# oscarkey/safe-exploration

Measured on AMD Instinct MI355X. Metric: cem_particle_step_evals_per_s, higher is better.
Workload: dtype f64

## Files before the change

safe_exploration_amd/csrc/sx_gp_rollout.hip:

```cpp
#include <hip/hip_runtime.h>

#include <algorithm>
#include <cstdlib>
#include <cstring>
#include <vector>

#include "../../include/sx_amd.h"
#include "sx_big.hpp"
#include "sx_big_launch.hpp"
#include "sx_host.hpp"
#include "sx_launch.hpp"
#include "sx_rw_launch.hpp"
#include "sx_stream_launch.hpp"

namespace sx {

#ifdef SX_STAMPS
extern unsigned long long* g_stamp_host;
#endif

struct RolloutPlan {
    int form;
    bool ok;
    size_t lds;
    int nrb;
};

struct FormOverride {
    int form;
    bool strict;
    bool refuses() const { return strict && form >= 0; }
};
static const FormOverride& form_override() {
    static const FormOverride o = [] {
        const char* e = std::getenv("SX_ROLLOUT");
        const int form = !e                            ? -1
                         : std::strcmp(e, "stream") == 0 ? SX_FORM_STREAM
                         : std::strcmp(e, "rw") == 0     ? SX_FORM_RW
                         : std::strcmp(e, "rh") == 0     ? SX_FORM_RH
                                                         : -1;
        return FormOverride{form, std::getenv("SX_ROLLOUT_STRICT") != nullptr};
    }();
    return o;
}

template <int NS, int NU>
static int resident_lds_bytes(int n_train, int n_pad, int H, size_t* rh, size_t* rw) {
    *rh = rollout_rh_lds_bytes<NS, NU>(n_train, n_pad, H);
    *rw = rollout_rw_lds_bytes<NS, NU>(n_train, n_pad, H);
    return SX_OK;
}
static int resident_lds_bytes(int ns, int nu, int n_train, int n_pad, int H, size_t* rh, size_t* rw) {
#define CALL(NS, NU) resident_lds_bytes<NS, NU>(n_train, n_pad, H, rh, rw)
    SX_DISPATCH(ns, nu, CALL);
#undef CALL
}

static RolloutPlan plan_rollout(const sx_gp_model* m, int sh, int H, bool elites, bool stream_only = false) {
    const int ns = m->n_s, nu = m->n_u - sh, n_train = m->n_train, n_pad = m->n_pad;
    auto stream_lds = [&](bool byout) { return rollout_stream_lds_bytes(ns, nu, sh, n_train, n_pad, H, byout); };
    const bool all_at_once = n_pad <= 1024 && stream_lds(false) <= kMaxLdsBytes;
    const bool by_output = !all_at_once && ns > 1 && n_pad <= 1024 && stream_lds(true) <= kMaxLdsBytes;
    bool ok = rollout_compiled(ns, nu, sh);
    if (!all_at_once && !by_output) return {SX_FORM_BIG, ok && sh == 0 && !elites, 0, 0};
    if (elites && 2 * H * nu > 256 + 256 * ns) ok = false;
    if (by_output) return {SX_FORM_BYOUT, ok, stream_lds(true), 0};
    const RolloutPlan stream{SX_FORM_STREAM, ok, stream_lds(false), 0};
    const FormOverride& o = form_override();
    if (!ok || sh > 0 || stream_only || o.form == SX_FORM_STREAM) return stream;
    size_t rh, rw;
    resident_lds_bytes(ns, nu, n_train, n_pad, H, &rh, &rw);
    if (o.form != SX_FORM_RW && rh <= kMaxLdsBytes) return {SX_FORM_RH, true, rh, n_pad >> 4};
    if (o.form != SX_FORM_RH && rw <= kMaxLdsBytes) return {SX_FORM_RW, true, rw, n_pad >> 4};
    return {SX_FORM_STREAM, !o.refuses(), stream.lds, 0};
}

template <int NS, int NU, int SH>
static int launch_rollout(const sx_gp_model* m, const sx_env* env, const RolloutPtrs& rp, double* workspace,
                          int64_t workspace_bytes, hipStream_t stream) {
    RolloutPlan plan = plan_rollout(m, SH, rp.H, rp.elite_rows != nullptr);
    if (!plan.ok) return SX_ERR_UNSUPPORTED;
    if constexpr (SH == 0) {
        if (plan.form == SX_FORM_BIG) return launch_rollout_big<NS, NU>(m, env, rp, workspace, workspace_bytes, stream);
    }
    ReachConst<NS, NU> rc;
    CostConst<SX_MAX_M, NS, NU> cc;
    if (int r = env_consts<NS, NU>(env, rc, cc)) return r;
    RolloutPtrs rps = rp;
#ifdef SX_STAMPS
    rps.stamps = g_stamp_host;
#endif
    if constexpr (SH == 0) {
        if (plan.form == SX_FORM_RH || plan.form == SX_FORM_RW) {
            const int r = plan.form == SX_FORM_RH
                              ? launch_rollout_rh<NS, NU>(make_gp_const<NS, NU>(m, 8), rc, cc, rps, plan.nrb, plan.lds, stream)
                              : launch_rollout_rw<NS, NU>(make_gp_const<NS, NU>(m, kRwWaves), rc, cc, rps, plan.nrb, plan.lds,
                                                          stream);
            if (r != SX_ERR_UNSUPPORTED || form_override().refuses()) return r;
            plan = {SX_FORM_STREAM, true, rollout_stream_lds_bytes(NS, NU, SH, m->n_train, m->n_pad, rp.H, false), 0};
        }
    }
    return launch_rollout_stream<NS, NU, SH>(make_gp_const<NS, NU + SH>(m, kRolloutThreads / 64), rc, cc, rps,
                                             plan.form == SX_FORM_BYOUT, plan.lds, stream);
}

static RolloutPlan plan_rollout_multi(const sx_gp_model* models, int E, int H, bool elites) {
    RolloutPlan out{SX_FORM_STREAM, true, 0, 0};
    for (int i = 0; i < E; ++i) {
        const RolloutPlan p = plan_rollout(&models[i], 0, H, elites, true);
        if (p.form == SX_FORM_BIG || !p.ok) return {p.form, false, 0, 0};
        if (p.form == SX_FORM_BYOUT) out.form = SX_FORM_BYOUT;
    }
    const sx_gp_model& m0 = models[0];
    for (int i = 0; i < E; ++i)
        out.lds = std::max(out.lds, rollout_stream_lds_bytes(m0.n_s, m0.n_u, 0, models[i].n_train, models[i].n_pad, H,
                                                             out.form == SX_FORM_BYOUT));
    return out;
}

template <int NS, int NU>
static int64_t gp_table_entry_bytes() {
    return (int64_t)sizeof(GpConst<NS, NS + NU>);
}
static int64_t gp_table_entry_bytes(int ns, int nu) {
#define CALL(NS, NU) gp_table_entry_bytes<NS, NU>()
    SX_DISPATCH(ns, nu, CALL);
#undef CALL
}

template <int NS, int NU>
static int build_gp_table(const sx_gp_model* models, int E, void* table, hipStream_t stream) {
    std::vector<GpConst<NS, NS + NU>> host(E);
    for (int i = 0; i < E; ++i) host[i] = make_gp_const<NS, NU>(&models[i], kRolloutThreads / 64);
    return copy_model_table(host, table, stream);
}

template <int NS, int NU>
static int launch_rollout_multi(const sx_gp_model* models, const void* table, const sx_env* env, const RolloutPtrs& rp,
                                hipStream_t stream) {
    const RolloutPlan plan = plan_rollout_multi(models, rp.E, rp.H, rp.elite_rows != nullptr);
    if (!plan.ok) return SX_ERR_UNSUPPORTED;
    ReachConst<NS, NU> rc;
    CostConst<SX_MAX_M, NS, NU> cc;
    if (int r = env_consts<NS, NU>(env, rc, cc)) return r;
    return launch_rollout_stream_multi<NS, NU>(static_cast<const GpConst<NS, NS + NU>*>(table), rc, cc, rp,
                                               plan.form == SX_FORM_BYOUT, plan.lds, stream);
}

static int cem_rollout(const sx_gp_model* model, const sx_env* env, int query_shift, const RolloutPtrs& rp, void* workspace,
                       int64_t workspace_bytes, void* stream) {
#define CALL(NS, NU, SH) launch_rollout<NS, NU, SH>(model, env, rp, (double*)workspace, workspace_bytes, (hipStream_t)stream)
    SX_ROLLOUT_DISPATCH(env->n_s, env->n_u, query_shift, CALL);
#undef CALL
}

}

extern "C" {

int64_t sx_cem_rollout_workspace_bytes(const sx_gp_model* model, int E, int P, int H) {
    if (!model || E <= 0 || P <= 0 || H <= 0) return -1;
    if (sx::plan_rollout(model, 0, H, false).form != SX_FORM_BIG) return 0;
    return sx::big_ws_layout(nullptr, model->n_s, model->n_s + model->n_u, model->n_pad, (int64_t)E * P).total *
           (int64_t)sizeof(double);
}

int sx_cem_rollout_form(const sx_gp_model* model, int H) {
    if (!model || H <= 0) return -1;
    const sx::RolloutPlan plan = sx::plan_rollout(model, 0, H, false);
    return plan.ok ? plan.form : -1;
}

int sx_cem_rollout(const sx_gp_model* model, const sx_env* env, int E, int P, int H, const double* x0, const double* q0,
                   const double* mean, const double* std, const double* noise, double* actions, double* traj,
                   double* sigma, double* obj_cost, double* con_cost, int32_t* status, void* workspace,
                   int64_t workspace_bytes, void* stream) {
    return sx_cem_rollout_junk(model, env, 0, E, P, H, x0, q0, mean, std, noise, actions, traj, sigma, obj_cost, con_cost,
                               status, workspace, workspace_bytes, stream);
}

int sx_cem_rollout_elites(const sx_gp_model* model, const sx_env* env, int E, int P, int H, const double* x0, const double* q0,
                          const double* elite_rows, int k, const double* noise, double* actions, double* traj, double* sigma,
                          double* obj_cost, double* con_cost, int32_t* status, double* mean_out, double* std_out, void* stream) {
    return sx_cem_rollout_elites_junk(model, env, 0, E, P, H, x0, q0, elite_rows, k, noise, actions, traj, sigma, obj_cost,
                                      con_cost, status, mean_out, std_out, stream);
}

static sx::RolloutPtrs with_elites(sx::RolloutPtrs rp, const double* elite_rows, int k, double* mean_out, double* std_out) {
    rp.elite_rows = elite_rows;
    rp.elite_k = k;
    rp.mean_out = mean_out;
    rp.std_out = std_out;
    return rp;
}

static bool rollout_shapes_ok(const sx_gp_model* model, const sx_env* env, int query_shift) {
    return model->n_s == env->n_s && query_shift >= 0 && query_shift <= env->n_u && model->n_u == env->n_u + query_shift;
}

int sx_cem_rollout_junk(const sx_gp_model* model, const sx_env* env, int query_shift, int E, int P, int H, const double* x0,
                        const double* q0, const double* mean, const double* std, const double* noise, double* actions,
                        double* traj, double* sigma, double* obj_cost, double* con_cost, int32_t* status, void* workspace,
                        int64_t workspace_bytes, void* stream) {
    const sx::RolloutPtrs rp{x0, q0, mean, std, noise, actions, traj, sigma, obj_cost, con_cost, status, E, P, H};
    if (!model || !sx::rollout_args_ok(env, rp) || !rollout_shapes_ok(model, env, query_shift)) return SX_ERR_ARG;
    return sx::cem_rollout(model, env, query_shift, rp, workspace, workspace_bytes, stream);
}

int sx_cem_rollout_elites_junk(const sx_gp_model* model, const sx_env* env, int query_shift, int E, int P, int H,
                               const double* x0, const double* q0, const double* elite_rows, int k, const double* noise,
                               double* actions, double* traj, double* sigma, double* obj_cost, double* con_cost,
                               int32_t* status, double* mean_out, double* std_out, void* stream) {
    const sx::RolloutPtrs rp = with_elites({x0, q0, nullptr, nullptr, noise, actions, traj, sigma, obj_cost, con_cost, status,
                                            E, P, H}, elite_rows, k, mean_out, std_out);
    if (!model || !elite_rows || !sx::rollout_args_ok(env, rp) || !rollout_shapes_ok(model, env, query_shift)) return SX_ERR_ARG;
    return sx::cem_rollout(model, env, query_shift, rp, nullptr, 0, stream);
}

static bool multi_models_ok(const sx_gp_model* models, int E) {
    if (!models || E <= 0) return false;
    const int ns = models[0].n_s, nu = models[0].n_u;
    if (ns <= 0 || ns > SX_MAX_NS || nu <= 0 || nu > SX_MAX_NU) return false;
    for (int i = 0; i < E; ++i)
        if (models[i].n_s != ns || models[i].n_u != nu || models[i].n_train <= 0 || models[i].n_pad <= 0) return false;
    return true;
}

int64_t sx_gp_model_table_bytes(int n_s, int n_u, int E) {
    if (E <= 0 || n_s <= 0 || n_s > SX_MAX_NS || n_u <= 0 || n_u > SX_MAX_NU) return -1;
    const int64_t entry = sx::gp_table_entry_bytes(n_s, n_u);
    return entry == SX_ERR_UNSUPPORTED ? -1 : entry * E;
}

int sx_gp_model_table(const sx_gp_model* models, int E, void* table, void* stream) {
    if (!table || !multi_models_ok(models, E)) return SX_ERR_ARG;
    for (int i = 0; i < E; ++i)
        if (!models[i].x_train || !models[i].a_pack || !models[i].stage_tab) return SX_ERR_ARG;
#define CALL(NS, NU) sx::build_gp_table<NS, NU>(models, E, table, (hipStream_t)stream)
    SX_DISPATCH(models[0].n_s, models[0].n_u, CALL);
#undef CALL
}

int sx_cem_rollout_multi_form(const sx_gp_model* models, int E, int H) {
    if (!multi_models_ok(models, E) || H <= 0) return -1;
    const sx::RolloutPlan plan = sx::plan_rollout_multi(models, E, H, false);
    return plan.ok ? plan.form : -1;
}

static int cem_rollout_multi(const sx_gp_model* models, const void* table, const sx_env* env, const sx::RolloutPtrs& rp,
                             void* stream) {
#define CALL(NS, NU) sx::launch_rollout_multi<NS, NU>(models, table, env, rp, (hipStream_t)stream)
    SX_DISPATCH(env->n_s, env->n_u, CALL);
#undef CALL
}

int sx_cem_rollout_multi(const sx_gp_model* models, const void* table, const sx_env* env, int E, int P, int H,
                         const double* x0, const double* q0, const double* mean, const double* std, const double* noise,
                         double* actions, double* traj, double* sigma, double* obj_cost, double* con_cost, int32_t* status,
                         void* stream) {
    const sx::RolloutPtrs rp{x0, q0, mean, std, noise, actions, traj, sigma, obj_cost, con_cost, status, E, P, H};
    if (!table || !sx::rollout_args_ok(env, rp) || !multi_models_ok(models, E)) return SX_ERR_ARG;
    if (models[0].n_s != env->n_s || models[0].n_u != env->n_u) return SX_ERR_ARG;
    return cem_rollout_multi(models, table, env, rp, stream);
}

int sx_cem_rollout_elites_multi(const sx_gp_model* models, const void* table, const sx_env* env, int E, int P, int H,
                                const double* x0, const double* q0, const double* elite_rows, int k, const double* noise,
                                double* actions, double* traj, double* sigma, double* obj_cost, double* con_cost,
                                int32_t* status, double* mean_out, double* std_out, void* stream) {
    const sx::RolloutPtrs rp = with_elites({x0, q0, nullptr, nullptr, noise, actions, traj, sigma, obj_cost, con_cost, status,
                                            E, P, H}, elite_rows, k, mean_out, std_out);
    if (!table || !elite_rows || !sx::rollout_args_ok(env, rp) || !multi_models_ok(models, E)) return SX_ERR_ARG;
    if (models[0].n_s != env->n_s || models[0].n_u != env->n_u) return SX_ERR_ARG;
    return cem_rollout_multi(models, table, env, rp, stream);
}

}
```

safe_exploration_amd/csrc/sx_rollout_rh.hpp:

```cpp
#pragma once
#include <hip/hip_runtime.h>

#include "../../include/sx_amd.h"
#include "sx_rollout_rw.hpp"

#ifndef SX_RH_REGP
#define SX_RH_REGP 26
#endif
#ifndef SX_RH_LEAD
#define SX_RH_LEAD -1
#endif
#ifndef SX_RH_LDSP
#define SX_RH_LDSP 8
#endif
#ifndef SX_RH_PFG
#define SX_RH_PFG 6
#endif
#ifndef SX_RH_PFL
#define SX_RH_PFL 2
#endif
#ifndef SX_RH_RBMAJOR
#define SX_RH_RBMAJOR 1
#endif
#ifndef SX_RH_PRIO
#define SX_RH_PRIO 0
#endif
#ifndef SX_RH_WFIRST
#define SX_RH_WFIRST 0
#endif
#ifndef SX_RH_SHARES
#define SX_RH_SHARES 4, 4, 4, 1, 4, 4, 4
#endif

namespace sx {

constexpr int kRhWaves = 8;
constexpr int kRhThreads = 64 * kRhWaves;

template <int NS, int NRB>
struct RhPlan {
    int wave_of[NS][NRB];
    int pairs[kRhWaves];
    constexpr RhPlan() : wave_of{}, pairs{} {
        for (int w = 0; w < kRhWaves; ++w) pairs[w] = 0;
        for (int d = 0; d < NS; ++d) {
            int lo = 0, n = kRhWaves;
            if (kRhWaves % NS == 0) {
                n = kRhWaves / NS;
                lo = d * n;
            }
            const bool rev = (kRhWaves % NS == 0) && (d & 1);
            int set_of[NRB] = {};
            int load[kRhWaves] = {};
            for (int rb = NRB - 1; rb >= 0; --rb) {
                int best = 0;
                for (int s = 1; s < n; ++s)
                    if (load[s] + pairs[lo + (rev ? n - 1 - s : s)] < load[best] + pairs[lo + (rev ? n - 1 - best : best)]) best = s;
                set_of[rb] = best;
                load[best] += 2 * (rb + 1);
            }
            for (int rb = 0; rb < NRB; ++rb) wave_of[d][rb] = lo + (rev ? n - 1 - set_of[rb] : set_of[rb]);
            for (int s = 0; s < n; ++s) pairs[lo + (rev ? n - 1 - s : s)] += load[s];
        }
    }
    constexpr int max_pairs() const {
        int m = 0;
        for (int w = 0; w < kRhWaves; ++w) m = pairs[w] > m ? pairs[w] : m;
        return m;
    }
    constexpr bool has(int w, int d) const {
        for (int rb = 0; rb < NRB; ++rb)
            if (wave_of[d][rb] == w) return true;
        return false;
    }
    constexpr int qmax(int w, int d) const {
        for (int rb = NRB - 1; rb >= 0; --rb)
            if (wave_of[d][rb] == w) return 2 * (rb + 1);
        return 0;
    }
};

template <int NS, int NRB>
struct RhElements {
    static constexpr int kMax = NS * NRB * (NRB + 1);
    short d[kRhWaves][kMax], rb[kRhWaves][kMax], q[kRhWaves][kMax];
    int n[kRhWaves];
    constexpr RhElements() : d{}, rb{}, q{}, n{} {
        const RhPlan<NS, NRB> plan{};
        for (int w = 0; w < kRhWaves; ++w) {
            int idx = 0;
            for (int dd = 0; dd < NS; ++dd) {
#if SX_RH_RBMAJOR
                for (int r = NRB - 1; r >= 0; --r)
                    for (int qq = 0; qq < 2 * (r + 1); ++qq)
                        if (plan.wave_of[dd][r] == w) { d[w][idx] = dd; rb[w][idx] = r; q[w][idx] = qq; ++idx; }
#else
                for (int qq = 0; qq < 2 * NRB; ++qq)
                    for (int r = NRB - 1; r >= 0; --r)
                        if (plan.wave_of[dd][r] == w && qq < 2 * (r + 1)) { d[w][idx] = dd; rb[w][idx] = r; q[w][idx] = qq; ++idx; }
#endif
            }
            n[w] = idx;
        }
    }
};

struct RhLayout {
    int nr, nl, ng, lead;
    constexpr RhLayout(int total, int regp, int ldsp)
        : nr(total < regp ? total : regp), nl(0), ng(0), lead(0) {
        nl = total - nr < ldsp ? total - nr : ldsp;
        ng = total - nr - nl;
        lead = SX_RH_LEAD < 0 || ng == 0 ? nr : (SX_RH_LEAD < nr ? SX_RH_LEAD : nr);
    }
    constexpr int storage(int e, int regp, int ldsp) const {
        if (SX_RH_LEAD < 0 || ng == 0) return e;
        if (e < lead) return e;
        if (e < lead + ng) return regp + ldsp + (e - lead);
        if (e < lead + ng + nl) return regp + (e - lead - ng);
        return lead + (e - lead - ng - nl);
    }
};

template <int NS, int NRB, int MAXP, int REGP, int LDSP>
struct RhStream {
    int pair[kRhWaves][MAXP];
    constexpr RhStream() : pair{} {
        const RhElements<NS, NRB> el{};
        constexpr int wpo = NRB * (NRB + 1);
        for (int w = 0; w < kRhWaves; ++w) {
            const RhLayout lay(el.n[w], REGP, LDSP);
            for (int i = 0; i < MAXP; ++i) pair[w][i] = 0;
            for (int e = 0; e < el.n[w]; ++e)
                pair[w][lay.storage(e, REGP, LDSP)] = el.d[w][e] * wpo + el.rb[w][e] * (el.rb[w][e] + 1) + el.q[w][e];
        }
    }
};

enum RhOpKind { kRhLoadB = 0, kRhLoadWL = 1, kRhLoadWG = 2, kRhMfma = 3, kRhRowEpi = 4, kRhFinalEpi = 5 };
struct RhOp {
    int kind;
    int i;
    int rb;
    int q;
    int d;
    int slot;
    int e;
};
template <int NS, int NRB, int WAVE, int REGP, int LDSP, int PF, int PFL, int PFG>
struct RhProgram {
    static constexpr int kMaxOps = 4 * NS * NRB * (NRB + 1) / 2 + 8 * NRB * NS + 16;
    RhOp ops[kMaxOps];
    int n;
    int total;
    constexpr RhProgram() : ops{}, n(0), total(0) {
        const RhElements<NS, NRB> el{};
        total = el.n[WAVE];
        const RhLayout lay(total, REGP, LDSP);
        int next_l = 0;
        int next_g = 0;
        const int e_g0 = (SX_RH_LEAD < 0 || lay.ng == 0) ? lay.nr + lay.nl : lay.lead;
        const int e_l0 = (SX_RH_LEAD < 0 || lay.ng == 0) ? lay.nr : lay.lead + lay.ng;
        int bslot[RhElements<NS, NRB>::kMax] = {};
        int bfirst[RhElements<NS, NRB>::kMax] = {};
        int nloads = 0;
        for (int e = 0; e < total; ++e) {
            const bool fresh = SX_RH_RBMAJOR || e == 0 || el.q[WAVE][e] != el.q[WAVE][e - 1] || el.d[WAVE][e] != el.d[WAVE][e - 1];
            if (fresh) ++nloads;
            bfirst[e] = fresh ? 1 : 0;
            bslot[e] = (nloads - 1) % (PF + 1);
        }
        constexpr int kDelay = 2;
        int pend_rb[NRB * NS] = {}, pend_d[NRB * NS] = {}, pend_at[NRB * NS] = {};
        int npend = 0, done = 0;
        int issued_b = 0;
        int eb = 0;
        auto issue_b_upto = [&](int loads_wanted) {
            while (issued_b < loads_wanted && eb < total) {
                if (bfirst[eb]) {
                    ops[n++] = RhOp{kRhLoadB, 0, 0, el.q[WAVE][eb], el.d[WAVE][eb], bslot[eb]};
                    ++issued_b;
                }
                ++eb;
            }
        };
        int loads_seen = 0;
        for (int e = 0; e < total; ++e) {
            if (bfirst[e]) ++loads_seen;
            issue_b_upto(loads_seen + PF);
            while (next_l < lay.nl && e_l0 + next_l <= e + PFL) ops[n++] = RhOp{kRhLoadWL, REGP + next_l++, 0, 0, 0, 0};
            while (next_g < lay.ng && e_g0 + next_g <= e + PFG) ops[n++] = RhOp{kRhLoadWG, REGP + LDSP + next_g++, 0, 0, 0, 0};
            ops[n++] = RhOp{kRhMfma, lay.storage(e, REGP, LDSP), el.rb[WAVE][e], el.q[WAVE][e], el.d[WAVE][e], bslot[e], e};
            const bool last_of_rb = el.q[WAVE][e] == 2 * (el.rb[WAVE][e] + 1) - 1;
            if (last_of_rb) {
                pend_rb[npend] = el.rb[WAVE][e];
                pend_d[npend] = el.d[WAVE][e];
                pend_at[npend] = e + kDelay;
                ++npend;
            }
            while (done < npend && pend_at[done] <= e) {
                ops[n++] = RhOp{kRhRowEpi, 0, pend_rb[done], 0, pend_d[done], 0};
                ++done;
            }
        }
        while (done < npend) {
            ops[n++] = RhOp{kRhRowEpi, 0, pend_rb[done], 0, pend_d[done], 0};
            ++done;
        }
        const RhPlan<NS, NRB> plan{};
        for (int d = 0; d < NS; ++d)
            if (plan.has(WAVE, d)) ops[n++] = RhOp{kRhFinalEpi, 0, 0, 0, d, 0};
    }
};

template <int NS, int D, int NRB, int WAVE, int REGP, int LDSP>
__device__ __forceinline__ void rh_mfma_phase(const GpConst<NS, D>& gc, GpTileLds<NS, D>& lds, const v2d* wlds_wave, int lane,
                                              const v2d (&wreg)[REGP]) {
    constexpr int PF = SX_RW_PF, PFL = SX_RH_PFL, PFG = SX_RH_PFG;
    constexpr int MAXP = RhPlan<NS, NRB>{}.max_pairs();
    static constexpr RhProgram<NS, NRB, WAVE, REGP, LDSP, PF, PFL, PFG> prog{};
    static constexpr RhStream<NS, NRB, MAXP, REGP, LDSP> stream{};
    const v2d* kbase = reinterpret_cast<const v2d*>(lds.kfrag) + lane;
    typedef const __attribute__((address_space(1))) v2d* gv2d;
    typedef const __attribute__((address_space(3))) v2d* lv2d;
    const v2d* ap_opaque = reinterpret_cast<const v2d*>(gc.a_pack) + lane;
    asm volatile("" : "+v"(ap_opaque));
    const gv2d ap = (gv2d)ap_opaque;
    const lv2d wl_base = (lv2d)wlds_wave + lane;
    v4d acc[NRB];
    v2d b[PF + 1];
    v2d wl[PFL + 1];
    v2d wg[PFG + 1];
    double ssq[NS];
#pragma unroll
    for (int d = 0; d < NS; ++d) ssq[d] = 0.0;
    static_for<0, prog.n>([&](auto ktag) {
        constexpr RhOp op = prog.ops[decltype(ktag)::value];
        if constexpr (op.kind == kRhLoadB) {
            b[op.slot] = kbase[(op.q * NS + op.d) * 64];
        } else if constexpr (op.kind == kRhLoadWL) {
            wl[op.i % (PFL + 1)] = wl_base[(op.i - REGP) * 64];
        } else if constexpr (op.kind == kRhLoadWG) {
            wg[op.i % (PFG + 1)] = ap[(size_t)stream.pair[WAVE][op.i] * 64];
        } else if constexpr (op.kind == kRhMfma) {
#if SX_RH_PRIO == 2
            if constexpr ((4 * op.e) / prog.total != (4 * (op.e - 1)) / prog.total || op.e == 0)
                __builtin_amdgcn_s_setprio(3 - (4 * op.e) / prog.total);
#endif
            SX_PIN();
            const v2d bq = b[op.slot];
            v2d a;
            if constexpr (op.i < REGP)
                a = wreg[op.i];
            else if constexpr (op.i < REGP + LDSP)
                a = wl[op.i % (PFL + 1)];
            else
                a = wg[op.i % (PFG + 1)];
            if constexpr (op.q == 0)
                acc[op.rb] = __builtin_amdgcn_mfma_f64_16x16x4f64(a.x, bq.x, v4d{0.0, 0.0, 0.0, 0.0}, 0, 0, 0);
            else
                acc[op.rb] = __builtin_amdgcn_mfma_f64_16x16x4f64(a.x, bq.x, acc[op.rb], 0, 0, 0);
            acc[op.rb] = __builtin_amdgcn_mfma_f64_16x16x4f64(a.y, bq.y, acc[op.rb], 0, 0, 0);
            SX_PIN();
        } else if constexpr (op.kind == kRhRowEpi) {
            constexpr int rb = op.rb, d = op.d;
            double s;
            if constexpr (rb >= NRB - 2) {
                const int row0 = rb * 16 + (lane >> 4);
                s = 0.0;
#pragma unroll
                for (int r = 0; r < 4; ++r) {
                    const int row = row0 + 4 * r;
                    if (row < gc.n_train)
                        s = fma(acc[rb][r], acc[rb][r], s);
                    else if (row - gc.n_train <= D)
                        lds.mj[d * 256 + (row - gc.n_train) * 16 + (lane & 15)] = acc[rb][r];
                }
            } else {
                s = fma(acc[rb][3], acc[rb][3], fma(acc[rb][2], acc[rb][2], fma(acc[rb][1], acc[rb][1], acc[rb][0] * acc[rb][0])));
            }
            ssq[d] += s;
        } else {
            constexpr int d = op.d;
            const v4d tot = __builtin_amdgcn_mfma_f64_16x16x4f64(1.0, ssq[d], v4d{0.0, 0.0, 0.0, 0.0}, 0, 0, 0);
            if (lane < 16) lds.part[(WAVE * NS + d) * 16 + lane] = tot[0];
        }
    });
}

template <int NS, int D, int NRB, bool WITH_JAC, typename G>
__device__ __forceinline__ void rh_collect(const G& gc, const GpTileLds<NS, D>& lds, int c, const double (&z)[D],
                                           double (&mean)[NS], double (&var)[NS], double (&jac)[NS][D]) {
    constexpr RhPlan<NS, NRB> plan{};
#pragma unroll
    for (int d = 0; d < NS; ++d) {
        double q = 0.0;
#pragma unroll
        for (int w = 0; w < kRhWaves; ++w)
            if (plan.has(w, d)) q += lds.part[(w * NS + d) * 16 + c];
        var[d] = (gc.outputscale[d] - q) + gc.noise[d];
        const double m = lds.mj[d * 256 + c];
        mean[d] = m;
        if constexpr (WITH_JAC) {
#pragma unroll
            for (int j = 0; j < D; ++j) jac[d][j] = lds.mj[d * 256 + (1 + j) * 16 + c] - z[j] * gc.inv_ls2[d * D + j] * m;
        }
    }
}

template <int NS, int NRB>
constexpr int rh_regp() {
    constexpr int m = RhPlan<NS, NRB>{}.max_pairs();
    return m < SX_RH_REGP ? m : SX_RH_REGP;
}
template <int NS, int NRB>
constexpr int rh_ldsp() {
    constexpr int rest = RhPlan<NS, NRB>{}.max_pairs() - rh_regp<NS, NRB>();
    return rest < SX_RH_LDSP ? rest : SX_RH_LDSP;
}
template <int NS, int NU, int NRB>
inline size_t rh_lds_doubles(int n_train, int n_pad, int H) {
    constexpr int D = NS + NU, S = NS + NS * NS;
    return (size_t)NS * n_pad * 16 + NS * 256 + (size_t)kRhWaves * NS * 16 + 32 * D + (((size_t)SX_TILE * H * NU + 1) & ~(size_t)1) +
           (((size_t)SX_TILE * (2 * (S + NS) + 3) + 1) & ~(size_t)1) + RwKstarLds<NS, D>::doubles(n_pad) +
           (size_t)kRhWaves * rh_ldsp<NS, NRB>() * 128;
}

template <int NS, int NU, int NRB>
__global__ __launch_bounds__(kRhThreads) void cem_rollout_rh_kernel(GpConst<NS, NS + NU> gc, ReachConst<NS, NU> rc,
                                                                    CostConst<SX_MAX_M, NS, NU> cc, RolloutPtrs rp) {
    constexpr int D = NS + NU;
    constexpr int S = NS + NS * NS;
    constexpr int PQS = S + NS;
    constexpr RhPlan<NS, NRB> plan{};
    constexpr int MAXP = plan.max_pairs();
    constexpr int REGP = rh_regp<NS, NRB>();
    constexpr int LDSP = rh_ldsp<NS, NRB>();
    extern __shared__ __attribute__((aligned(16))) double smem[];
    GpTileLds<NS, D> lds;
    constexpr int nw = kRhWaves;
    lds.xs = nullptr;
    lds.etab = nullptr;
    lds.kfrag = smem;
    lds.mj = lds.kfrag + (size_t)NS * gc.n_pad * 16;
    lds.part = lds.mj + NS * 256;
    lds.zs = lds.part + (size_t)nw * NS * 16;
    double* acts = lds.zs + 32 * D;
    const int tid = threadIdx.x;
    const int wave = __builtin_amdgcn_readfirstlane(tid >> 6), lane = tid & 63;
    const int H = rp.H;
    const int tiles_per_problem = (rp.P + SX_TILE - 1) / SX_TILE;
    const int total_tiles = rp.E * tiles_per_problem;

    RwConst<NS, NU>* const cst = reinterpret_cast<RwConst<NS, NU>*>(acts + (((size_t)SX_TILE * rp.H * NU + 1) & ~(size_t)1));
    double* const pq = reinterpret_cast<double*>(cst + 1);
    RwKstarLds<NS, D> kl;
    kl.carve(pq + (((size_t)SX_TILE * (2 * PQS + 3) + 1) & ~(size_t)1), gc.n_pad);
    v2d* const wlds = reinterpret_cast<v2d*>(kl.xbar + ((D + 1) & ~1));

    static constexpr RhStream<NS, NRB, MAXP, REGP, LDSP> stream{};
    v2d wreg[REGP];
#if SX_RH_WFIRST
    {
        const v2d* __restrict__ const ap0 = reinterpret_cast<const v2d*>(gc.a_pack) + lane;
#pragma unroll
        for (int i = 0; i < REGP; ++i) wreg[i] = ap0[(size_t)stream.pair[wave][i] * 64];
        if constexpr (LDSP > 0) {
#pragma unroll
            for (int i = 0; i < LDSP; ++i) wlds[(wave * LDSP + i) * 64 + lane] = ap0[(size_t)stream.pair[wave][REGP + i] * 64];
        }
    }
#endif
    {
        static_assert(sizeof(RwConst<NS, NU>) % 8 == 0 && sizeof(ReachConst<NS, NU>) % 8 == 0 &&
                      sizeof(CostConst<SX_MAX_M, NS, NU>) % 8 == 0, "copied in 8-byte words");
        constexpr int nrc = sizeof(ReachConst<NS, NU>) / 8, ncc = sizeof(CostConst<SX_MAX_M, NS, NU>) / 8;
        double* dst = reinterpret_cast<double*>(cst);
        const double* src_rc = reinterpret_cast<const double*>(&rc);
        const double* src_cc = reinterpret_cast<const double*>(&cc);
        for (int i = tid; i < nrc; i += kRhThreads) dst[i] = src_rc[i];
        for (int i = tid; i < ncc; i += kRhThreads) dst[nrc + i] = src_cc[i];
        if (tid < NS * D) cst->inv_ls2[tid] = gc.inv_ls2[tid];
        if (tid < NS) {
            cst->outputscale[tid] = gc.outputscale[tid];
            cst->noise[tid] = gc.noise[tid];
        }
    }
    const RwConst<NS, NU>& fc = *cst;
    const ReachConst<NS, NU>& frc = cst->rc;
    const CostConst<SX_MAX_M, NS, NU>& fcc = cst->cc;
    rw_kstar_setup(gc, kl, lds.kfrag);
    const int kstar_pairs = (gc.n_train + 7) >> 3;

    const bool owner = tid < SX_TILE;
    int q0_begin, q0_end, q_begin = 0, q_end = 0;
    kstar_pair_range(kstar_pairs, wave, 1, nw, q0_begin, q0_end);
    if (wave > 0) {
        constexpr int kShare[8] = {0, SX_RH_SHARES};
        int before = 0, total = 0;
#pragma unroll
        for (int w = 1; w < 8; ++w) {
            if (w < wave) before += kShare[w];
            total += kShare[w];
        }
        kstar_pair_range(kstar_pairs, before, kShare[wave], total, q_begin, q_end);
    }
    double* const zs_base = lds.zs;

    for (int tile = blockIdx.x; tile < total_tiles; tile += gridDim.x) {
#ifdef SX_STAMPS
        const unsigned long long tile_t0 = stamp();
        unsigned long long first_k = 0, first_kb = 0;
#endif
        const int e = tile / tiles_per_problem;
        const int c0 = (tile - e * tiles_per_problem) * SX_TILE;
        const bool valid = owner && (c0 + tid < rp.P);

        const double* dist_mean = rp.mean + (int64_t)e * H * NU;
        const double* dist_std = rp.std + (int64_t)e * H * NU;
        bool have_q = rp.q0 != nullptr;
        if (rp.elite_rows) {
            const int L = H * NU, W = 2 + L;
            double* const ms = lds.kfrag;
            const double* rows = rp.elite_rows + (int64_t)e * rp.elite_k * W + 2;
            const bool publish = c0 == 0 && rp.mean_out;
            int cshift = 0;
            while ((nw << cshift) < L && cshift < 6) ++cshift;
            const int ccol = lane & ((1 << cshift) - 1);
            for (int cb = wave << cshift; cb < L; cb += nw << cshift) {
                const int col = cb + ccol;
                double m, sd;
                wave_refit_columns(rows + (col < L ? col : L - 1), rp.elite_k, W, lane, cshift, m, sd);
                if ((lane >> cshift) == 0 && col < L) {
                    ms[col] = m;
                    ms[L + col] = sd;
                    if (publish) {
                        rp.mean_out[(int64_t)e * L + col] = m;
                        rp.std_out[(int64_t)e * L + col] = sd;
                    }
                }
            }
            __syncthreads();
            dist_mean = ms;
            dist_std = ms + L;
        }
        for (int i = tid; i < SX_TILE * H * NU; i += kRhThreads) {
            const int c = i / (H * NU);
            const int r = i - c * (H * NU);
            double a = 0.0;
            if (c0 + c < rp.P) {
                const int64_t gi = ((int64_t)e * rp.P + c0 + c) * (H * NU) + r;
                if (rp.noise) {
                    a = dist_mean[r] + dist_std[r] * rp.noise[gi];
                    rp.actions[gi] = a;
                } else {
                    a = rp.actions[gi];
                }
            }
            acts[i] = a;
        }
        const bool lane_owner = lane < SX_TILE;
        const bool lane_valid = lane_owner && (c0 + lane < rp.P);
        auto st_row = [&](int buf, int c) { return pq + (buf * SX_TILE + c) * PQS; };
        double* const ac_row = pq + 2 * SX_TILE * PQS + (lane_owner ? lane : 0) * 3;
        if (owner) {
            double* my = st_row(0, tid);
#pragma unroll
            for (int i = 0; i < NS; ++i) {
                my[i] = rp.x0[(int64_t)e * NS + i];
#pragma unroll
                for (int j = 0; j < NS; ++j) my[NS + i * NS + j] = have_q ? rp.q0[((int64_t)e * NS + i) * NS + j] : 0.0;
            }
            ac_row[0] = 0.0;
            ac_row[1] = 0.0;
            reinterpret_cast<int*>(ac_row + 2)[0] = 0;
        }
        __syncthreads();
        if (owner) {
            const double* my = st_row(0, tid);
#pragma unroll
            for (int i = 0; i < NS; ++i) lds.zs[tid * D + i] = my[i];
#pragma unroll
            for (int cidx = 0; cidx < NU; ++cidx) lds.zs[tid * D + NS + cidx] = acts[(tid * H + 0) * NU + cidx];
        }
        __syncthreads();

        if (!SX_RH_WFIRST && tile == (int)blockIdx.x) {
            const v2d* __restrict__ const ap = reinterpret_cast<const v2d*>(gc.a_pack) + lane;
            if constexpr (LDSP > 0) {
                const __amdgpu_buffer_rsrc_t arsrc =
                    __builtin_amdgcn_make_buffer_rsrc(const_cast<double*>(gc.a_pack), 0, (int)0xffffffffu, 0x00020000);
#pragma unroll
                for (int i = 0; i < LDSP; ++i) {
                    const int pair = __builtin_amdgcn_readfirstlane(stream.pair[wave][REGP + i]);
                    __builtin_amdgcn_raw_ptr_buffer_load_lds(
                        arsrc, (__attribute__((address_space(3))) void*)(wlds + (wave * LDSP + i) * 64), 16, lane * 16, pair << 10, 0, 0);
                }
            }
#pragma unroll
            for (int i = 0; i < REGP; ++i) wreg[i] = ap[(size_t)stream.pair[wave][i] * 64];
        }

        auto next_centre = [&](const ReachConst<NS, NU>& R, int c, const double* z_prev, double (&out)[NS]) {
#pragma unroll
            for (int i = 0; i < NS; ++i) {
                double s = lds.mj[i * 256 + c];
#pragma unroll
                for (int j = 0; j < NS; ++j) s = fma(R.a[i * NS + j], z_prev[j], s);
#pragma unroll
                for (int cidx = 0; cidx < NU; ++cidx) s = fma(R.b[i * NU + cidx], z_prev[NS + cidx], s);
                out[i] = s;
            }
        };
        auto finish_state = [&](int t) {
            double z[D], u[NU], mean[NS], var[NS], jac[NS][D], p1[NS], Q1[NS][NS];
            double p[NS], Q[NS][NS];
            constexpr RhPlan<NS, NRB> plan{};
            const double* my = st_row(t & 1, lane);
            double partv[NS][kRhWaves], mjv[NS][1 + D], ils2[NS][D], osc[NS], nzv[NS];
#pragma unroll
            for (int d = 0; d < NS; ++d) {
#pragma unroll
                for (int w = 0; w < kRhWaves; ++w) partv[d][w] = plan.has(w, d) ? lds.part[(w * NS + d) * 16 + lane] : 0.0;
#pragma unroll
                for (int r = 0; r < 1 + D; ++r) mjv[d][r] = lds.mj[d * 256 + r * 16 + lane];
            }
#pragma unroll
            for (int i = 0; i < NS; ++i) {
                p[i] = my[i];
#pragma unroll
                for (int j = 0; j < NS; ++j) Q[i][j] = my[NS + i * NS + j];
            }
#pragma unroll
            for (int cidx = 0; cidx < NU; ++cidx) u[cidx] = acts[(lane * H + t) * NU + cidx];
#pragma unroll
            for (int d = 0; d < NS; ++d) {
                osc[d] = fc.outputscale[d];
                nzv[d] = fc.noise[d];
#pragma unroll
                for (int j = 0; j < D; ++j) ils2[d][j] = fc.inv_ls2[d * D + j];
            }
            SX_PIN();
            const ReachConst<NS, NU>& rcv = frc;
#pragma unroll
            for (int j = 0; j < NS; ++j) z[j] = p[j];
#pragma unroll
            for (int cidx = 0; cidx < NU; ++cidx) z[NS + cidx] = u[cidx];
#pragma unroll
            for (int d = 0; d < NS; ++d) {
                double q = 0.0;
#pragma unroll
                for (int w = 0; w < kRhWaves; ++w)
                    if (plan.has(w, d)) q += partv[d][w];
                var[d] = (osc[d] - q) + nzv[d];
                mean[d] = mjv[d][0];
#pragma unroll
                for (int j = 0; j < D; ++j) jac[d][j] = mjv[d][1 + j] - z[j] * ils2[d][j] * mean[d];
            }
            int st_step = 0;
            if (have_q) {
                reach_ellipsoid<NS, NU>(rcv, p, Q, u, mean, var, jac, p1, Q1, st_step);
            } else {
                reach_point<NS, NU>(rcv, p, u, mean, var, p1, Q1, st_step);
            }
            have_q = true;
            {
                double zt[D];
#pragma unroll
                for (int j = 0; j < NS; ++j) zt[j] = p[j];
#pragma unroll
                for (int cidx = 0; cidx < NU; ++cidx) zt[NS + cidx] = u[cidx];
#pragma unroll
                for (int i = 0; i < NS; ++i) {
                    double sc = mean[i];
#pragma unroll
                    for (int j = 0; j < NS; ++j) sc = fma(rcv.a[i * NS + j], zt[j], sc);
#pragma unroll
                    for (int cidx = 0; cidx < NU; ++cidx) sc = fma(rcv.b[i * NU + cidx], zt[NS + cidx], sc);
                    p1[i] = sc;
                }
                if (t + 1 < H) {
                    double* zn = zs_base + ((t + 1) & 1) * 16 * D + lane * D;
#pragma unroll
                    for (int i = 0; i < NS; ++i) zn[i] = p1[i];
#pragma unroll
                    for (int cidx = 0; cidx < NU; ++cidx) zn[NS + cidx] = acts[(lane * H + t + 1) * NU + cidx];
                }
            }
            if (lane_valid && st_step) reinterpret_cast<int*>(ac_row + 2)[0] |= st_step;
            double* nx = st_row((t + 1) & 1, lane);
#pragma unroll
            for (int i = 0; i < NS; ++i) {
                nx[i] = p1[i];
#pragma unroll
                for (int j = 0; j < NS; ++j) nx[NS + i * NS + j] = Q1[i][j];
                nx[S + i] = var[i];
            }
        };
        auto finish_costs = [&](int t) {
            const int c = lane & 15;
            const double* o = st_row((t + 1) & 1, c);
            double pp[NS], QQ[NS][NS], var[NS], hrow[NS], hv, uu[NU], umin[NU], umax[NU], wab[NS], tgt[NS], wli[NS];
            const int m = fcc.m, obj_mode = fcc.obj_mode, con_mode = fcc.con_mode;
            const int r0 = lane >> 4;
            const int r0c = r0 < m ? r0 : 0;
#pragma unroll
            for (int i = 0; i < NS; ++i) {
                pp[i] = o[i];
#pragma unroll
                for (int j = 0; j < NS; ++j) QQ[i][j] = o[NS + i * NS + j];
                var[i] = o[S + i];
                hrow[i] = fcc.h_mat[r0c * NS + i];
                wab[i] = fcc.w_abs[i];
                tgt[i] = fcc.target[i];
                wli[i] = fcc.w_lin[i];
            }
            hv = fcc.h_vec[r0c];
#pragma unroll
            for (int cidx = 0; cidx < NU; ++cidx) {
                uu[cidx] = acts[(c * H + t) * NU + cidx];
                umin[cidx] = fcc.u_min[cidx];
                umax[cidx] = fcc.u_max[cidx];
            }
            double obj = ac_row[0], con = ac_row[1];
            SX_PIN();
            bool viol = false;
            if (con_mode == SX_CON_ALL_STATES || t == H - 1) {
                for (int r = r0; r < m; r += 4) {
                    if (r != r0) {
#pragma unroll
                        for (int i = 0; i < NS; ++i) hrow[i] = fcc.h_mat[r * NS + i];
                        hv = fcc.h_vec[r];
                    }
                    double hc = 0.0, hq = 0.0;
#pragma unroll
                    for (int i = 0; i < NS; ++i) {
                        hc += hrow[i] * pp[i];
                        double sacc = 0.0;
#pragma unroll
                        for (int j = 0; j < NS; ++j) sacc += QQ[i][j] * hrow[j];
                        hq += hrow[i] * sacc;
                    }
                    const double dist = hc + sqrt(hq) - hv;
                    viol = viol || (dist >= 0.0);
                }
            }
            unsigned long long bits = __ballot(viol);
            bits |= bits >> 32;
            bits |= bits >> 16;
            if (lane_owner) {
                if ((bits >> lane) & 1ull) con += SX_STATE_VIOLATION_COST;
                bool uviol = false;
#pragma unroll
                for (int cidx = 0; cidx < NU; ++cidx) uviol = uviol || (uu[cidx] < umin[cidx]) || (uu[cidx] > umax[cidx]);
                if (uviol) con += SX_ACTION_VIOLATION_COST;
                double oadd = 0.0;
                if (obj_mode == SX_OBJ_NEG_VARIANCE) {
#pragma unroll
                    for (int i = 0; i < NS; ++i) oadd -= var[i];
                } else {
#pragma unroll
                    for (int i = 0; i < NS; ++i) oadd += wab[i] * fabs(tgt[i] - pp[i]) + wli[i] * pp[i];
                }
                obj += oadd;
                ac_row[0] = obj;
                ac_row[1] = con;
                const int64_t g = (int64_t)e * rp.P + c0 + lane;
                if (lane_valid && rp.traj) {
                    double* tr = rp.traj + (g * H + t) * S;
#pragma unroll
                    for (int i = 0; i < NS; ++i) {
                        tr[i] = pp[i];
#pragma unroll
                        for (int j = 0; j < NS; ++j) tr[NS + i * NS + j] = QQ[i][j];
                    }
                }
                if (lane_valid && rp.sigma) {
#pragma unroll
                    for (int i = 0; i < NS; ++i) rp.sigma[(g * H + t) * NS + i] = var[i];
                }
            }
        };

#ifdef SX_STAMPS
        unsigned long long c_k = 0, c_kb = 0, c_m = 0, c_mb = 0;
        unsigned long long rt0;
        asm volatile("s_memrealtime %0\n\ts_waitcnt lgkmcnt(0)" : "=s"(rt0)::"memory");
        const unsigned long long ct0 = stamp();
#endif
        for (int t = 0; t < H; ++t) {
#ifdef SX_STAMPS
            const unsigned long long t0 = stamp();
#endif
            const bool kstar_wave = !(t > 0 && wave == 0);
            if (wave == 4 && t > 1) finish_costs(t - 2);
            if (kstar_wave) {
                double zq[D];
                const int c = lane & 15;
                if (t == 0) {
#pragma unroll
                    for (int j = 0; j < D; ++j) zq[j] = zs_base[c * D + j];
                    rw_kstar_phase(gc, kl, lds.kfrag, q0_begin, q0_end, zq);
                } else {
                    double pc[NS];
                    next_centre(rc, c, zs_base + ((t - 1) & 1) * 16 * D + c * D, pc);
#pragma unroll
                    for (int i = 0; i < NS; ++i) zq[i] = pc[i];
#pragma unroll
                    for (int cidx = 0; cidx < NU; ++cidx) zq[NS + cidx] = acts[(c * H + t) * NU + cidx];
                    rw_kstar_phase(gc, kl, lds.kfrag, q_begin, q_end, zq);
                }
            } else if (owner) {
                finish_state(t - 1);
            }
#ifdef SX_STAMPS
            const unsigned long long t1 = stamp();
#endif
            if (t == 0) asm volatile("s_waitcnt vmcnt(0)" ::: "memory");
            __syncthreads();
#ifdef SX_STAMPS
            const unsigned long long t2 = stamp();
#endif
            const v2d* wl = wlds + wave * LDSP * 64;
#if SX_RH_PRIO == 1
            if (wave < 4) __builtin_amdgcn_s_setprio(3);
#endif
            switch (wave) {
                case 0: rh_mfma_phase<NS, D, NRB, 0, REGP, LDSP>(gc, lds, wl, lane, wreg); break;
                case 1: rh_mfma_phase<NS, D, NRB, 1, REGP, LDSP>(gc, lds, wl, lane, wreg); break;
                case 2: rh_mfma_phase<NS, D, NRB, 2, REGP, LDSP>(gc, lds, wl, lane, wreg); break;
                case 3: rh_mfma_phase<NS, D, NRB, 3, REGP, LDSP>(gc, lds, wl, lane, wreg); break;
                case 4: rh_mfma_phase<NS, D, NRB, 4, REGP, LDSP>(gc, lds, wl, lane, wreg); break;
                case 5: rh_mfma_phase<NS, D, NRB, 5, REGP, LDSP>(gc, lds, wl, lane, wreg); break;
                case 6: rh_mfma_phase<NS, D, NRB, 6, REGP, LDSP>(gc, lds, wl, lane, wreg); break;
                default: rh_mfma_phase<NS, D, NRB, 7, REGP, LDSP>(gc, lds, wl, lane, wreg); break;
            }
#if SX_RH_PRIO == 1
            if (wave < 4) __builtin_amdgcn_s_setprio(0);
#elif SX_RH_PRIO == 2
            __builtin_amdgcn_s_setprio(0);
#endif
#ifdef SX_STAMPS
            const unsigned long long t3 = stamp();
#endif
            __syncthreads();
#ifdef SX_STAMPS
            const unsigned long long t4 = stamp();
            c_k += t1 - t0; c_kb += t2 - t1; c_m += t3 - t2; c_mb += t4 - t3;
            if (t == 0) { first_k = t1 - t0; first_kb = t2 - t1; }
#endif
        }
#ifdef SX_STAMPS
        const unsigned long long loop_t1 = stamp();
        if (rp.stamps && lane == 0 && tile == (int)blockIdx.x) {
            unsigned long long* o = rp.stamps + ((size_t)blockIdx.x * nw + wave) * 8;
            o[0] = c_k; o[1] = c_kb; o[2] = c_m; o[3] = c_mb;
            o[4] = (ct0 - tile_t0) | (first_k << 32);
            unsigned long long rt1;
            asm volatile("s_memrealtime %0\n\ts_waitcnt lgkmcnt(0)" : "=s"(rt1)::"memory");
            o[6] = stamp() - ct0;
            o[7] = rt1 - rt0;
        }
#endif
        if (wave == 0 && owner) finish_state(H - 1);
        if (wave == 4 && H > 1) finish_costs(H - 2);
        __syncthreads();
        if (wave == 0) finish_costs(H - 1);
        if (valid) {
            const int64_t g = (int64_t)e * rp.P + c0 + tid;
            rp.obj_cost[g] = ac_row[0];
            rp.con_cost[g] = ac_row[1];
            const int st = reinterpret_cast<const int*>(ac_row + 2)[0];
            if (st) atomicOr(rp.status, st);
        }
        __syncthreads();
#ifdef SX_STAMPS
        if (rp.stamps && lane == 0 && tile == (int)blockIdx.x)
            rp.stamps[((size_t)blockIdx.x * nw + wave) * 8 + 5] = (stamp() - loop_t1) | (first_kb << 32);
#endif
    }
}

}
```

safe_exploration_amd/csrc/sx_rollout_rw.hpp:

```cpp
#pragma once
#include <hip/hip_runtime.h>

#include "../../include/sx_amd.h"
#include "sx_exp2_tab2048.hpp"
#include "sx_gp.hpp"
#include "sx_reach.hpp"
#include "sx_refit.hpp"
#include "sx_rollout.hpp"
#include "sx_rw_launch.hpp"

#ifndef SX_RW_LDSCONST
#define SX_RW_LDSCONST 1
#endif
#ifndef SX_RW_POLYLANES
#define SX_RW_POLYLANES 1
#endif
#ifndef SX_RW_PF
#define SX_RW_PF 2
#endif
#ifndef SX_RW_RCLOCAL
#define SX_RW_RCLOCAL 0
#endif
#ifndef SX_RW_POLYFOLD
#define SX_RW_POLYFOLD 0
#endif

namespace sx {

constexpr int kRwThreads = 64 * kRwWaves;
constexpr int kRwMaxPairs = 93;

template <int B, int E, typename F>
__device__ __forceinline__ void static_for(F&& f) {
    if constexpr (B < E) {
        f(std::integral_constant<int, B>{});
        static_for<B + 1, E>(f);
    }
}

template <int NS, int NRB>
struct RwPlan {
    int wave_of[NS][NRB];
    int pairs[kRwWaves];
    constexpr RwPlan() : wave_of{}, pairs{} {
        for (int w = 0; w < kRwWaves; ++w) pairs[w] = 0;
        for (int rb = NRB - 1; rb >= 0; --rb)
            for (int d = 0; d < NS; ++d) {
                int lo = 0, hi = kRwWaves;
                if (kRwWaves % NS == 0) {
                    lo = d * (kRwWaves / NS);
                    hi = lo + kRwWaves / NS;
                }
                int best = lo;
                for (int w = lo + 1; w < hi; ++w)
                    if (pairs[w] < pairs[best]) best = w;
                wave_of[d][rb] = best;
                pairs[best] += 2 * (rb + 1);
            }
    }
    constexpr int max_pairs() const {
        int m = 0;
        for (int w = 0; w < kRwWaves; ++w) m = pairs[w] > m ? pairs[w] : m;
        return m;
    }
    constexpr bool has(int w, int d) const {
        for (int rb = 0; rb < NRB; ++rb)
            if (wave_of[d][rb] == w) return true;
        return false;
    }
    constexpr int qmax(int w, int d) const {
        for (int rb = NRB - 1; rb >= 0; --rb)
            if (wave_of[d][rb] == w) return 2 * (rb + 1);
        return 0;
    }
};

template <int NS, int NRB>
constexpr bool rw_fits() {
    return RwPlan<NS, NRB>{}.max_pairs() <= kRwMaxPairs;
}

template <int NS, int NRB, int MAXP>
struct RwLoadTab {
    int pair[kRwWaves][MAXP];
    constexpr RwLoadTab() : pair{} {
        const RwPlan<NS, NRB> plan{};
        constexpr int wpo = NRB * (NRB + 1);
        for (int w = 0; w < kRwWaves; ++w) {
            int idx = 0;
            for (int d = 0; d < NS; ++d)
                for (int rb = NRB - 1; rb >= 0; --rb) {
                    if (plan.wave_of[d][rb] != w) continue;
                    for (int q = 0; q < 2 * (rb + 1); ++q) pair[w][idx++] = d * wpo + rb * (rb + 1) + q;
                }
            for (; idx < MAXP; ++idx) pair[w][idx] = 0;
        }
    }
};

template <int NS, int D, int NRB, int MAXP>
__device__ __forceinline__ void rw_load_w(const GpConst<NS, D>& gc, int wave, int lane, v2d (&wreg)[MAXP]) {
    static constexpr RwLoadTab<NS, NRB, MAXP> tab{};
    const v2d* __restrict__ ap = reinterpret_cast<const v2d*>(gc.a_pack) + lane;
#pragma unroll
    for (int i = 0; i < MAXP; ++i) wreg[i] = ap[(size_t)tab.pair[wave][i] * 64];
}

template <int NS, int D, int NRB, int WAVE, int MAXP, int PF = SX_RW_PF>
__device__ __forceinline__ void rw_mfma_phase(const GpConst<NS, D>& gc, GpTileLds<NS, D>& lds, int lane,
                                              const v2d (&wreg)[MAXP]) {
    constexpr RwPlan<NS, NRB> plan{};
    const v2d* kbase = reinterpret_cast<const v2d*>(lds.kfrag) + lane;
    int first[NS][NRB];
    {
        int idx = 0;
#pragma unroll
        for (int d = 0; d < NS; ++d)
#pragma unroll
            for (int rb = NRB - 1; rb >= 0; --rb) {
                first[d][rb] = idx;
                if (plan.wave_of[d][rb] == WAVE) idx += 2 * (rb + 1);
            }
    }
    static_for<0, NS>([&](auto dtag) {
        constexpr int d = decltype(dtag)::value;
        constexpr int qmax = plan.qmax(WAVE, d);
        if constexpr (qmax > 0) {
        v4d acc[NRB];
        v2d b[PF + 1];
#pragma unroll
        for (int q = 0; q < PF && q < qmax; ++q) b[q] = kbase[(q * NS + d) * 64];
#pragma unroll
        for (int q = 0; q < qmax; ++q) {
            if (q + PF < qmax) b[(q + PF) % (PF + 1)] = kbase[((q + PF) * NS + d) * 64];
            SX_PIN();
            const v2d bq = b[q % (PF + 1)];
#pragma unroll
            for (int rb = NRB - 1; rb >= 0; --rb) {
                if (plan.wave_of[d][rb] != WAVE || q >= 2 * (rb + 1)) continue;
                const v2d a = wreg[first[d][rb] + q];
                if (q == 0)
                    acc[rb] = __builtin_amdgcn_mfma_f64_16x16x4f64(a.x, bq.x, v4d{0.0, 0.0, 0.0, 0.0}, 0, 0, 0);
                else
                    acc[rb] = __builtin_amdgcn_mfma_f64_16x16x4f64(a.x, bq.x, acc[rb], 0, 0, 0);
                acc[rb] = __builtin_amdgcn_mfma_f64_16x16x4f64(a.y, bq.y, acc[rb], 0, 0, 0);
            }
            SX_PIN();
        }
        double ssq = 0.0;
#pragma unroll
        for (int rb = NRB - 1; rb >= 0; --rb) {
            if (plan.wave_of[d][rb] != WAVE) continue;
            double s;
            if (rb >= NRB - 2) {
                const int row0 = rb * 16 + (lane >> 4);
                s = 0.0;
#pragma unroll
                for (int r = 0; r < 4; ++r) {
                    const int row = row0 + 4 * r;
                    if (row < gc.n_train)
                        s = fma(acc[rb][r], acc[rb][r], s);
                    else if (row - gc.n_train <= D)
                        lds.mj[d * 256 + (row - gc.n_train) * 16 + (lane & 15)] = acc[rb][r];
                }
            } else {
                s = fma(acc[rb][3], acc[rb][3], fma(acc[rb][2], acc[rb][2], fma(acc[rb][1], acc[rb][1], acc[rb][0] * acc[rb][0])));
            }
            ssq += s;
        }
        const v4d tot = __builtin_amdgcn_mfma_f64_16x16x4f64(1.0, ssq, v4d{0.0, 0.0, 0.0, 0.0}, 0, 0, 0);
        if (lane < 16) lds.part[(WAVE * NS + d) * 16 + lane] = tot[0];
        }
    });
}

constexpr double kExpScale2 = 2048.0 / 0.693147180559945309417232;
constexpr double kExpUnit2 = 0.693147180559945309417232 / 2048.0;

template <int NS, int D>
struct RwKstarLds {
    double* rows;
    double* tab;
    double* xbar;
    static __host__ __device__ size_t doubles(int n_pad) { return (size_t)n_pad * (D + NS) + (n_pad & 1) + kExpTab2 + 2 + ((D + 1) & ~1); }
    __device__ void carve(double* base, int n_pad) {
        rows = base;
        tab = rows + (size_t)n_pad * (D + NS) + (n_pad & 1);
        xbar = tab + kExpTab2 + 2;
    }
};

template <int NS, int D>
__device__ __forceinline__ void rw_kstar_setup(const GpConst<NS, D>& gc, const RwKstarLds<NS, D>& kl, double* kfrag) {
    const int tid = threadIdx.x, lane = tid & 63;
    double xb[D];
#pragma unroll
    for (int j = 0; j < D; ++j) {
        double v = lane < gc.n_train ? gc.x_train[lane * D + j] : 0.0;
        for (int off = 32; off > 0; off >>= 1) v += __shfl_xor(v, off);
        xb[j] = v / (double)(gc.n_train < 64 ? gc.n_train : 64);
        if (tid == 0) kl.xbar[j] = xb[j];
    }
    for (int k = tid; k < gc.n_pad; k += blockDim.x) {
        double xr[D], cc[NS];
#pragma unroll
        for (int d = 0; d < NS; ++d) cc[d] = 0.0;
#pragma unroll
        for (int j = 0; j < D; ++j) {
            xr[j] = k < gc.n_train ? gc.x_train[k * D + j] - xb[j] : 0.0;
#pragma unroll
            for (int d = 0; d < NS; ++d) cc[d] = fma(gc.k_nh_ils2[d * D + j], xr[j] * xr[j], cc[d]);
        }
#pragma unroll
        for (int j = 0; j < D; ++j) kl.rows[k * (D + NS) + j] = xr[j];
#pragma unroll
        for (int d = 0; d < NS; ++d) kl.rows[k * (D + NS) + D + d] = cc[d];
    }
    for (int i = tid; i < kExpTab2; i += blockDim.x) kl.tab[i] = kExp2Tab2048[i];
    if (tid < 2) kl.tab[kExpTab2 + tid] = __builtin_nan("");
    const int first_pad = ((gc.n_train + 7) >> 3) * NS * 128;
    for (int i = first_pad + tid; i < (gc.n_pad >> 3) * NS * 128; i += blockDim.x) kfrag[i] = 0.0;
}

template <int NS, int D>
__device__ __forceinline__ void rw_kstar_phase(const GpConst<NS, D>& gc, const RwKstarLds<NS, D>& kl, double* kfrag,
                                               int q_begin, int q_end, const double (&z)[D]) {
    constexpr int M = 2 * NS, RS = D + NS;
    const int n = q_end - q_begin;
    if (n <= 0) return;
    const int lane = (int)threadIdx.x & 63;
    const int c = lane & 15;
    double zz[NS], g[NS][D];
    bool znan = false;
    {
        double zc[D];
#pragma unroll
        for (int j = 0; j < D; ++j) {
            zc[j] = z[j] - kl.xbar[j];
            znan = znan || (z[j] != z[j]);
        }
#pragma unroll
        for (int d = 0; d < NS; ++d) {
            double a = gc.k_log_os[d];
#pragma unroll
            for (int j = 0; j < D; ++j) {
                const double kz = gc.k_nh_ils2[d * D + j] * zc[j];
                a = fma(kz, zc[j], a);
                g[d][j] = -2.0 * kz;
            }
            zz[d] = a;
        }
    }
    const lds_f64* etab = (const lds_f64*)kl.tab + (znan ? kExpTab2 : 0);
    const int emask = znan ? 0 : kExpTab2 - 1;
    const int k0 = 8 * q_begin + (lane >> 4);
    const lds_f64* x = (const lds_f64*)kl.rows + k0 * RS;
    lds_f64* f = (lds_f64*)kfrag + kfrag_index(NS, c, k0, 0);

    struct Set {
        double t[M], p[M];
        int mi[M];
    };
    auto load_x = [&](double (&xx)[2 * RS]) {
        asm volatile("" : "+v"(x));
#pragma unroll
        for (int h = 0; h < 2; ++h)
#pragma unroll
            for (int j = 0; j < RS; ++j) xx[h * RS + j] = x[h * 4 * RS + j];
        x += 8 * RS;
    };
    auto stage_a1 = [&](const double (&xx)[2 * RS], Set& s) {
        double yc[M], m[M];
#pragma unroll
        for (int h = 0; h < 2; ++h)
#pragma unroll
            for (int d = 0; d < NS; ++d) {
                double a = xx[h * RS + D + d] + zz[d];
#pragma unroll
                for (int j = 0; j < D; ++j) a = fma(g[d][j], xx[h * RS + j], a);
                yc[h * NS + d] = a;
            }
#pragma unroll
        for (int i = 0; i < M; ++i) yc[i] = __builtin_fmax(yc[i], -800.0 * kExpScale2);
#pragma unroll
        for (int i = 0; i < M; ++i) m[i] = __builtin_rint(yc[i]);
#pragma unroll
        for (int i = 0; i < M; ++i) asm("v_cvt_i32_f64 %0, %1" : "=v"(s.mi[i]) : "v"(m[i]));
#pragma unroll
        for (int i = 0; i < M; ++i) s.t[i] = etab[s.mi[i] & emask];
#pragma unroll
#if SX_RW_POLYFOLD
        for (int i = 0; i < M; ++i) s.p[i] = yc[i] - m[i];
#else
        for (int i = 0; i < M; ++i) s.p[i] = (yc[i] - m[i]) * kExpUnit2;
#endif
    };
    auto stage_a2 = [&](Set& s) {
        double r[M];
#pragma unroll
        for (int i = 0; i < M; ++i) r[i] = s.p[i];
#pragma unroll
#if SX_RW_POLYFOLD
        for (int i = 0; i < M; ++i) s.p[i] = fma(r[i], kExpUnit2 * kExpUnit2 * kExpUnit2 / 6.0, kExpUnit2 * kExpUnit2 * 0.5);
#pragma unroll
        for (int i = 0; i < M; ++i) s.p[i] = fma(s.p[i], r[i], kExpUnit2);
#else
        for (int i = 0; i < M; ++i) s.p[i] = fma(r[i], 1.66666666666666666667e-01, 0.5);
#pragma unroll
        for (int i = 0; i < M; ++i) s.p[i] = fma(s.p[i], r[i], 1.0);
#endif
#pragma unroll
        for (int i = 0; i < M; ++i) s.p[i] = s.p[i] * r[i];
    };
    auto stage_b = [&](const Set& s) {
        asm volatile("" : "+v"(f));
        double val[M];
#pragma unroll
        for (int i = 0; i < M; ++i) val[i] = ldexp(fma(s.t[i], s.p[i], s.t[i]), s.mi[i] >> 11);
#pragma unroll
        for (int d = 0; d < NS; ++d) {
            f[d * 128] = val[d];
            f[d * 128 + 1] = val[NS + d];
        }
        f += NS * 128;
    };
    double xr[2 * RS];
    Set s0, s1;
    load_x(xr);
    stage_a1(xr, s0);
    load_x(xr);
    stage_a2(s0);
    auto body = [&](const Set& sold, Set& snew) {
        stage_a1(xr, snew);
        SX_PIN();
        load_x(xr);
        stage_b(sold);
        SX_PIN();
        stage_a2(snew);
        SX_PIN();
    };
    const int n1 = n - 1;
    for (int k = 0; k < (n1 >> 1); ++k) {
        body(s0, s1);
        body(s1, s0);
    }
    if (n1 & 1) {
        body(s0, s1);
        stage_b(s1);
    } else {
        stage_b(s0);
    }
}

template <int NS, int NU>
struct alignas(16) RwConst {
    ReachConst<NS, NU> rc;
    CostConst<SX_MAX_M, NS, NU> cc;
    double inv_ls2[NS * (NS + NU)];
    double outputscale[NS];
    double noise[NS];
};

template <int NS, int D, int NRB, bool WITH_JAC, typename G>
__device__ __forceinline__ void rw_collect(const G& gc, const GpTileLds<NS, D>& lds, int c,
                                           const double (&z)[D], double (&mean)[NS], double (&var)[NS],
                                           double (&jac)[NS][D]) {
    constexpr RwPlan<NS, NRB> plan{};
#pragma unroll
    for (int d = 0; d < NS; ++d) {
        double q = 0.0;
#pragma unroll
        for (int w = 0; w < kRwWaves; ++w)
            if (plan.has(w, d)) q += lds.part[(w * NS + d) * 16 + c];
        var[d] = (gc.outputscale[d] - q) + gc.noise[d];
        const double m = lds.mj[d * 256 + c];
        mean[d] = m;
        if constexpr (WITH_JAC) {
#pragma unroll
            for (int j = 0; j < D; ++j) jac[d][j] = lds.mj[d * 256 + (1 + j) * 16 + c] - z[j] * gc.inv_ls2[d * D + j] * m;
        }
    }
}

template <int NS, int NU, int NRB>
__global__ __launch_bounds__(kRwThreads) __attribute__((amdgpu_waves_per_eu(1, 1)))
void cem_rollout_rw_kernel(GpConst<NS, NS + NU> gc, ReachConst<NS, NU> rc, CostConst<SX_MAX_M, NS, NU> cc, RolloutPtrs rp) {
    constexpr int D = NS + NU;
    constexpr int S = NS + NS * NS;
    constexpr int PQS = S + 3;
    constexpr RwPlan<NS, NRB> plan{};
    constexpr int MAXP = plan.max_pairs();
    static_assert(MAXP <= kRwMaxPairs, "W does not fit the register budget");
    extern __shared__ __attribute__((aligned(16))) double smem[];
    GpTileLds<NS, D> lds;
    constexpr int nw = kRwWaves;
    double* acts = lds.carve(smem, gc.n_train, gc.n_pad, nw, NS);
    const int tid = threadIdx.x;
#if SX_RW_LDSCONST
    RwConst<NS, NU>* const cst = reinterpret_cast<RwConst<NS, NU>*>(acts + (((size_t)SX_TILE * rp.H * NU + 1) & ~(size_t)1));
    {
        static_assert(sizeof(RwConst<NS, NU>) % 8 == 0 && sizeof(ReachConst<NS, NU>) % 8 == 0 &&
                      sizeof(CostConst<SX_MAX_M, NS, NU>) % 8 == 0, "copied in 8-byte words");
        constexpr int nrc = sizeof(ReachConst<NS, NU>) / 8, ncc = sizeof(CostConst<SX_MAX_M, NS, NU>) / 8;
        double* dst = reinterpret_cast<double*>(cst);
        const double* src_rc = reinterpret_cast<const double*>(&rc);
        const double* src_cc = reinterpret_cast<const double*>(&cc);
        for (int i = tid; i < nrc; i += kRwThreads) dst[i] = src_rc[i];
        for (int i = tid; i < ncc; i += kRwThreads) dst[nrc + i] = src_cc[i];
        if (tid < NS * D) cst->inv_ls2[tid] = gc.inv_ls2[tid];
        if (tid < NS) {
            cst->outputscale[tid] = gc.outputscale[tid];
            cst->noise[tid] = gc.noise[tid];
        }
    }
    double* const pq = reinterpret_cast<double*>(cst + 1);
    const RwConst<NS, NU>& fc = *cst;
    const ReachConst<NS, NU>& frc = cst->rc;
    const CostConst<SX_MAX_M, NS, NU>& fcc = cst->cc;
#else
    double* const pq = acts + (((size_t)SX_TILE * rp.H * NU + 1) & ~(size_t)1);
    const GpConst<NS, D>& fc = gc;
    const ReachConst<NS, NU>& frc = rc;
    const CostConst<SX_MAX_M, NS, NU>& fcc = cc;
#endif
    const int wave = __builtin_amdgcn_readfirstlane(tid >> 6), lane = tid & 63;
    const int H = rp.H;
    const int tiles_per_problem = (rp.P + SX_TILE - 1) / SX_TILE;
    const int total_tiles = rp.E * tiles_per_problem;

    v2d wreg[MAXP];
    rw_load_w<NS, D, NRB>(gc, wave, lane, wreg);
    RwKstarLds<NS, D> kl;
    kl.carve(pq + (((size_t)SX_TILE * PQS + 1) & ~(size_t)1), gc.n_pad);
    rw_kstar_setup(gc, kl, lds.kfrag);
    const int kstar_pairs = (gc.n_train + 7) >> 3;

    const bool owner = tid < SX_TILE;
    int q0_begin, q0_end, q_begin = 0, q_end = 0;
    kstar_pair_range(kstar_pairs, wave, 1, nw, q0_begin, q0_end);
    if (wave > 0) kstar_pair_range(kstar_pairs, wave - 1, 1, nw - 1, q_begin, q_end);
    double* const zs_base = lds.zs;

    for (int tile = blockIdx.x; tile < total_tiles; tile += gridDim.x) {
        const int e = tile / tiles_per_problem;
        const int c0 = (tile - e * tiles_per_problem) * SX_TILE;
        const bool valid = owner && (c0 + tid < rp.P);

        const double* dist_mean = rp.mean + (int64_t)e * H * NU;
        const double* dist_std = rp.std + (int64_t)e * H * NU;
        if (rp.elite_rows) {
            const int L = H * NU, W = 2 + L;
            double* const ms = lds.kfrag;
            const double* rows = rp.elite_rows + (int64_t)e * rp.elite_k * W + 2;
            const bool publish = c0 == 0 && rp.mean_out;
            int cshift = 0;
            while ((nw << cshift) < L && cshift < 6) ++cshift;
            const int ccol = lane & ((1 << cshift) - 1);
            for (int cb = wave << cshift; cb < L; cb += nw << cshift) {
                const int col = cb + ccol;
                double m, sd;
                wave_refit_columns(rows + (col < L ? col : L - 1), rp.elite_k, W, lane, cshift, m, sd);
                if ((lane >> cshift) == 0 && col < L) {
                    ms[col] = m;
                    ms[L + col] = sd;
                    if (publish) {
                        rp.mean_out[(int64_t)e * L + col] = m;
                        rp.std_out[(int64_t)e * L + col] = sd;
                    }
                }
            }
            __syncthreads();
            dist_mean = ms;
            dist_std = ms + L;
        }
        for (int i = tid; i < SX_TILE * H * NU; i += kRwThreads) {
            const int c = i / (H * NU);
            const int r = i - c * (H * NU);
            double a = 0.0;
            if (c0 + c < rp.P) {
                const int64_t gi = ((int64_t)e * rp.P + c0 + c) * (H * NU) + r;
                if (rp.noise) {
                    a = dist_mean[r] + dist_std[r] * rp.noise[gi];
                    rp.actions[gi] = a;
                } else {
                    a = rp.actions[gi];
                }
            }
            acts[i] = a;
        }
        bool have_q = rp.q0 != nullptr;
        double* const my = pq + (owner ? tid : 0) * PQS;
#ifdef SX_STAMPS
        unsigned long long c_f_collect = 0, c_f_reach = 0;
#endif
        if (owner) {
#pragma unroll
            for (int i = 0; i < NS; ++i) {
                my[i] = rp.x0[(int64_t)e * NS + i];
#pragma unroll
                for (int j = 0; j < NS; ++j) my[NS + i * NS + j] = have_q ? rp.q0[((int64_t)e * NS + i) * NS + j] : 0.0;
            }
            my[S] = 0.0;
            my[S + 1] = 0.0;
            reinterpret_cast<int*>(my + S + 2)[0] = 0;
        }
        __syncthreads();
        if (owner) {
#pragma unroll
            for (int i = 0; i < NS; ++i) lds.zs[tid * D + i] = my[i];
#pragma unroll
            for (int cidx = 0; cidx < NU; ++cidx) lds.zs[tid * D + NS + cidx] = acts[(tid * H + 0) * NU + cidx];
        }
        __syncthreads();

        auto next_centre = [&](const ReachConst<NS, NU>& R, int c, const double* z_prev, double (&out)[NS]) {
#pragma unroll
            for (int i = 0; i < NS; ++i) {
                double s = lds.mj[i * 256 + c];
#pragma unroll
                for (int j = 0; j < NS; ++j) s = fma(R.a[i * NS + j], z_prev[j], s);
#pragma unroll
                for (int cidx = 0; cidx < NU; ++cidx) s = fma(R.b[i * NU + cidx], z_prev[NS + cidx], s);
                out[i] = s;
            }
        };
        auto finish = [&](int t) {
            double z[D], u[NU], mean[NS], var[NS], jac[NS][D], p1[NS], Q1[NS][NS];
            double p[NS], Q[NS][NS];
#pragma unroll
            for (int i = 0; i < NS; ++i) {
                p[i] = my[i];
#pragma unroll
                for (int j = 0; j < NS; ++j) Q[i][j] = my[NS + i * NS + j];
            }
            double obj = my[S], con = my[S + 1];
#pragma unroll
            for (int j = 0; j < NS; ++j) z[j] = p[j];
#pragma unroll
            for (int cidx = 0; cidx < NU; ++cidx) {
                u[cidx] = acts[(tid * H + t) * NU + cidx];
                z[NS + cidx] = u[cidx];
            }
            int st_step = 0;
            if (have_q) {
#ifdef SX_STAMPS
                const unsigned long long f0 = stamp();
#endif
                rw_collect<NS, D, NRB, true>(fc, lds, tid, z, mean, var, jac);
#ifdef SX_STAMPS
                const unsigned long long f1 = stamp();
#endif
#if SX_RW_RCLOCAL
                if constexpr (NS >= 3) {
                    const ReachConst<NS, NU> rloc = frc;
                    SX_PIN();
                    reach_ellipsoid<NS, NU>(rloc, p, Q, u, mean, var, jac, p1, Q1, st_step);
                } else
#endif
                reach_ellipsoid<NS, NU>(frc, p, Q, u, mean, var, jac, p1, Q1, st_step);
#ifdef SX_STAMPS
                c_f_collect += f1 - f0;
                c_f_reach += stamp() - f1;
#endif
            } else {
                rw_collect<NS, D, NRB, false>(fc, lds, tid, z, mean, var, jac);
                reach_point<NS, NU>(frc, p, u, mean, var, p1, Q1, st_step);
            }
            have_q = true;
            {
                double zt[D];
#pragma unroll
                for (int j = 0; j < NS; ++j) zt[j] = p[j];
#pragma unroll
                for (int cidx = 0; cidx < NU; ++cidx) zt[NS + cidx] = u[cidx];
                next_centre(frc, tid, zt, p1);
                if (t + 1 < H) {
                    double* zn = zs_base + ((t + 1) & 1) * 16 * D + tid * D;
#pragma unroll
                    for (int i = 0; i < NS; ++i) zn[i] = p1[i];
#pragma unroll
                    for (int cidx = 0; cidx < NU; ++cidx) zn[NS + cidx] = acts[(tid * H + t + 1) * NU + cidx];
                }
            }
            if (valid && st_step) reinterpret_cast<int*>(my + S + 2)[0] |= st_step;
            obj += objective_cost<SX_MAX_M, NS, NU>(fcc, p1, var);
            bool uviol = false;
#pragma unroll
            for (int cidx = 0; cidx < NU; ++cidx) uviol = uviol || (u[cidx] < fcc.u_min[cidx]) || (u[cidx] > fcc.u_max[cidx]);
            if (uviol) con += SX_ACTION_VIOLATION_COST;
#if !SX_RW_POLYLANES
            if (fcc.con_mode == SX_CON_ALL_STATES || t == H - 1) {
                if (polytope_violated<SX_MAX_M, NS>(fcc.h_mat, fcc.h_vec, fcc.m, 1.0, p1, Q1, nullptr))
                    con += SX_STATE_VIOLATION_COST;
            }
#endif
#pragma unroll
            for (int i = 0; i < NS; ++i) {
                my[i] = p1[i];
#pragma unroll
                for (int j = 0; j < NS; ++j) my[NS + i * NS + j] = Q1[i][j];
            }
            my[S] = obj;
            my[S + 1] = con;
            const int64_t g = (int64_t)e * rp.P + c0 + tid;
            if (valid && rp.traj) {
                double* tr = rp.traj + (g * H + t) * S;
#pragma unroll
                for (int i = 0; i < NS; ++i) {
                    tr[i] = p1[i];
#pragma unroll
                    for (int j = 0; j < NS; ++j) tr[NS + i * NS + j] = Q1[i][j];
                }
            }
            if (valid && rp.sigma) {
#pragma unroll
                for (int i = 0; i < NS; ++i) rp.sigma[(g * H + t) * NS + i] = var[i];
            }
        };

#if SX_RW_POLYLANES
        auto finish_polytope = [&](int t) {
            if (!(fcc.con_mode == SX_CON_ALL_STATES || t == H - 1)) return;
            const int c = lane & 15;
            const double* o = pq + c * PQS;
            double pp[NS], QQ[NS][NS];
#pragma unroll
            for (int i = 0; i < NS; ++i) {
                pp[i] = o[i];
#pragma unroll
                for (int j = 0; j < NS; ++j) QQ[i][j] = o[NS + i * NS + j];
            }
            bool viol = false;
            const int m = fcc.m;
            for (int r = lane >> 4; r < m; r += 4) {
                double hc = 0.0, hq = 0.0;
#pragma unroll
                for (int i = 0; i < NS; ++i) {
                    const double hi = fcc.h_mat[r * NS + i];
                    hc += hi * pp[i];
                    double sacc = 0.0;
#pragma unroll
                    for (int j = 0; j < NS; ++j) sacc += QQ[i][j] * fcc.h_mat[r * NS + j];
                    hq += hi * sacc;
                }
                const double dist = hc + sqrt(hq) - fcc.h_vec[r];
                viol = viol || (dist >= 0.0);
            }
            unsigned long long bits = __ballot(viol);
            bits |= bits >> 32;
            bits |= bits >> 16;
            if (owner && ((bits >> tid) & 1ull)) my[S + 1] += SX_STATE_VIOLATION_COST;
        };
#else
        auto finish_polytope = [&](int) {};
#endif

#ifdef SX_STAMPS
        unsigned long long c_k = 0, c_kb = 0, c_m = 0, c_mb = 0;
        c_f_collect = c_f_reach = 0;
        unsigned long long rt0;
        asm volatile("s_memrealtime %0\n\ts_waitcnt lgkmcnt(0)" : "=s"(rt0)::"memory");
        const unsigned long long ct0 = stamp();
#endif
        for (int t = 0; t < H; ++t) {
#ifdef SX_STAMPS
            const unsigned long long t0 = stamp();
#endif
            const bool kstar_wave = !(t > 0 && wave == 0);
            if (kstar_wave) {
                double zq[D];
                const int c = lane & 15;
                if (t == 0) {
#pragma unroll
                    for (int j = 0; j < D; ++j) zq[j] = zs_base[c * D + j];
                    rw_kstar_phase(gc, kl, lds.kfrag, q0_begin, q0_end, zq);
                } else {
                    double pc[NS];
                    next_centre(rc, c, zs_base + ((t - 1) & 1) * 16 * D + c * D, pc);
#pragma unroll
                    for (int i = 0; i < NS; ++i) zq[i] = pc[i];
#pragma unroll
                    for (int cidx = 0; cidx < NU; ++cidx) zq[NS + cidx] = acts[(c * H + t) * NU + cidx];
                    rw_kstar_phase(gc, kl, lds.kfrag, q_begin, q_end, zq);
                }
            } else {
                if (owner) finish(t - 1);
                finish_polytope(t - 1);
            }
#ifdef SX_STAMPS
            const unsigned long long t1 = stamp();
#endif
            __syncthreads();
#ifdef SX_STAMPS
            const unsigned long long t2 = stamp();
#endif
            switch (wave) {
                case 0: rw_mfma_phase<NS, D, NRB, 0>(gc, lds, lane, wreg); break;
                case 1: rw_mfma_phase<NS, D, NRB, 1>(gc, lds, lane, wreg); break;
                case 2: rw_mfma_phase<NS, D, NRB, 2>(gc, lds, lane, wreg); break;
                default: rw_mfma_phase<NS, D, NRB, 3>(gc, lds, lane, wreg); break;
            }
#ifdef SX_STAMPS
            const unsigned long long t3 = stamp();
#endif
            __syncthreads();
#ifdef SX_STAMPS
            const unsigned long long t4 = stamp();
            c_k += t1 - t0; c_kb += t2 - t1; c_m += t3 - t2; c_mb += t4 - t3;
#endif
        }
#ifdef SX_STAMPS
        if (rp.stamps && lane == 0 && tile == (int)blockIdx.x) {
            unsigned long long* o = rp.stamps + ((size_t)blockIdx.x * nw + wave) * 8;
            o[0] = c_k; o[1] = c_kb; o[2] = c_m; o[3] = c_mb; o[4] = c_f_collect; o[5] = c_f_reach;
            unsigned long long rt1;
            asm volatile("s_memrealtime %0\n\ts_waitcnt lgkmcnt(0)" : "=s"(rt1)::"memory");
            o[6] = stamp() - ct0;
            o[7] = rt1 - rt0;
        }
#endif
        if (owner) finish(H - 1);
        if (wave == 0) finish_polytope(H - 1);
        if (valid) {
            const int64_t g = (int64_t)e * rp.P + c0 + tid;
            rp.obj_cost[g] = my[S];
            rp.con_cost[g] = my[S + 1];
            const int st = reinterpret_cast<const int*>(my + S + 2)[0];
            if (st) atomicOr(rp.status, st);
        }
        __syncthreads();
    }
}

}
```

safe_exploration_amd/csrc/sx_rw_impl.hpp:

```cpp
#pragma once
#include <type_traits>

#include "sx_launch.hpp"
#include "sx_rollout_rh.hpp"
#include "sx_rollout_rw.hpp"
#include "sx_rw_launch.hpp"

namespace sx {

template <int MAX, typename R, typename F>
static R with_nrb(int nrb, R none, F&& f) {
    if constexpr (MAX == 0) {
        return none;
    } else {
        if (nrb == MAX) return f(std::integral_constant<int, MAX>{});
        return with_nrb<MAX - 1>(nrb, none, f);
    }
}

template <int NS, int NU>
size_t rollout_rh_lds_bytes(int n_train, int n_pad, int H) {
    return with_nrb<rh_max_nrb(NS, NU)>(n_pad >> 4, ~(size_t)0, [&](auto nrb_c) {
        return rh_lds_doubles<NS, NU, decltype(nrb_c)::value>(n_train, n_pad, H) * sizeof(double) + sizeof(RwConst<NS, NU>);
    });
}

template <int NS, int NU>
size_t rollout_rw_lds_bytes(int n_train, int n_pad, int H) {
    const int nrb = n_pad >> 4;
    if (nrb < 1 || nrb > rw_max_nrb(NS, NU)) return ~(size_t)0;
    return (gp_tile_lds_doubles(NS, NS + NU, n_train, n_pad, kRwWaves, NS) + (((size_t)SX_TILE * H * NU + 1) & ~(size_t)1) +
            (((size_t)SX_TILE * (NS + NS * NS + 3) + 1) & ~(size_t)1) + RwKstarLds<NS, NS + NU>::doubles(n_pad)) *
               sizeof(double) +
           sizeof(RwConst<NS, NU>);
}

template <int NS, int D>
static GpConst<NS, D> in_exp2_2048_units(const GpConst<NS, D>& gc) {
    GpConst<NS, D> g8 = gc;
    for (int i = 0; i < NS * D; ++i) g8.k_nh_ils2[i] *= 8.0;
    for (int d = 0; d < NS; ++d) g8.k_log_os[d] *= 8.0;
    return g8;
}

static int resident_grid(const RolloutPtrs& rp) {
    const int tiles = rp.E * ((rp.P + SX_TILE - 1) / SX_TILE);
    return tiles < device_cus() ? tiles : device_cus();
}

template <int NS, int NU>
int launch_rollout_rh(const GpConst<NS, NS + NU>& gc, const ReachConst<NS, NU>& rc, const CostConst<SX_MAX_M, NS, NU>& cc,
                      const RolloutPtrs& rp, int nrb, size_t lds, hipStream_t stream) {
    const GpConst<NS, NS + NU> g8 = in_exp2_2048_units(gc);
    return with_nrb<rh_max_nrb(NS, NU)>(nrb, (int)SX_ERR_UNSUPPORTED, [&](auto nrb_c) {
        constexpr int NRB = decltype(nrb_c)::value;
        if (int r = allow_lds(cem_rollout_rh_kernel<NS, NU, NRB>, lds)) return r;
        launch(SX_PROF_ROLLOUT_FUSED, cem_rollout_rh_kernel<NS, NU, NRB>, dim3(resident_grid(rp)), dim3(kRhThreads), lds, stream,
               g8, rc, cc, rp);
        return check_launch();
    });
}

template <int NS, int NU>
int launch_rollout_rw(const GpConst<NS, NS + NU>& gc, const ReachConst<NS, NU>& rc, const CostConst<SX_MAX_M, NS, NU>& cc,
                      const RolloutPtrs& rp, int nrb, size_t lds, hipStream_t stream) {
    const GpConst<NS, NS + NU> g8 = in_exp2_2048_units(gc);
    return with_nrb<rw_max_nrb(NS, NU)>(nrb, (int)SX_ERR_UNSUPPORTED, [&](auto nrb_c) {
        constexpr int NRB = decltype(nrb_c)::value;
        static_assert(rw_fits<NS, NRB>(), "rw_max_nrb promises more than the register budget holds");
        if (int r = allow_lds(cem_rollout_rw_kernel<NS, NU, NRB>, lds)) return r;
        launch(SX_PROF_ROLLOUT_FUSED, cem_rollout_rw_kernel<NS, NU, NRB>, dim3(resident_grid(rp)), dim3(kRwThreads), lds, stream,
               g8, rc, cc, rp);
        return check_launch();
    });
}

}

#define SX_RW_INSTANTIATE(NS, NU)                                                                                         \
    template size_t rollout_rh_lds_bytes<NS, NU>(int, int, int);                                                          \
    template size_t rollout_rw_lds_bytes<NS, NU>(int, int, int);                                                          \
    template int launch_rollout_rh<NS, NU>(const GpConst<NS, NS + NU>&, const ReachConst<NS, NU>&,                        \
                                           const CostConst<SX_MAX_M, NS, NU>&, const RolloutPtrs&, int, size_t, hipStream_t); \
    template int launch_rollout_rw<NS, NU>(const GpConst<NS, NS + NU>&, const ReachConst<NS, NU>&,                        \
                                           const CostConst<SX_MAX_M, NS, NU>&, const RolloutPtrs&, int, size_t, hipStream_t);
```

safe_exploration_amd/csrc/sx_rw_launch.hpp:

```cpp
#pragma once
#include <hip/hip_runtime.h>

#include "../../include/sx_amd.h"
#include "sx_gp.hpp"
#include "sx_reach.hpp"
#include "sx_rollout.hpp"

namespace sx {

constexpr int kRwWaves = 4;

constexpr int rw_max_nrb(int ns, int nu) {
    return ns == 1 ? 18 : ns == 2 ? (nu == 1 ? 13 : 12) : ns == 3 ? 8 : (nu == 1 ? 6 : 5);
}


constexpr int rh_max_nrb(int ns, int nu) { return ns == 1 ? 18 : ns == 2 ? (nu == 1 ? 13 : 8) : 0; }

template <int NS, int NU>
size_t rollout_rh_lds_bytes(int n_train, int n_pad, int H);
template <int NS, int NU>
size_t rollout_rw_lds_bytes(int n_train, int n_pad, int H);

template <int NS, int NU>
int launch_rollout_rh(const GpConst<NS, NS + NU>& gc, const ReachConst<NS, NU>& rc, const CostConst<SX_MAX_M, NS, NU>& cc,
                      const RolloutPtrs& rp, int nrb, size_t lds, hipStream_t stream);
template <int NS, int NU>
int launch_rollout_rw(const GpConst<NS, NS + NU>& gc, const ReachConst<NS, NU>& rc, const CostConst<SX_MAX_M, NS, NU>& cc,
                      const RolloutPtrs& rp, int nrb, size_t lds, hipStream_t stream);

}
```

Baseline: 464.2 million.

## Overlap next-step k* query setup in an idle producer wave via LDS flags

Adds an LDS flag protocol: waves that own the mean-row blocks signal when their results are written, and a designated producer wave that owns no mean rows polls those flags. Once they are set, it precomputes the next step's kernel query (centred z, exponent base and gradients) into an LDS record during the MFMA phase. It also replaces the per-wave MFMA reduction of the sum of squares with raw per-lane partial stores that the consumer sums itself, and removes the old priority and wave-first options. This is meant to hide the serial query setup behind matrix work. In exchange it uses more LDS, adds spin-polling with a fallback marker, and brings a subtle cross-wave synchronisation risk.

```diff
diff --git a/safe_exploration_amd/csrc/sx_gp_rollout.hip b/safe_exploration_amd/csrc/sx_gp_rollout.hip
--- a/safe_exploration_amd/csrc/sx_gp_rollout.hip
+++ b/safe_exploration_amd/csrc/sx_gp_rollout.hip
@@ -54,6 +54,22 @@
 #define CALL(NS, NU) resident_lds_bytes<NS, NU>(n_train, n_pad, H, rh, rw)
     SX_DISPATCH(ns, nu, CALL);
 #undef CALL
+}
+
+template <int NS, int NU>
+static int rh_carved_bytes(int n_pad, int H, size_t* out) {
+    *out = rollout_rh_carved_bytes<NS, NU>(n_pad, H);
+    return SX_OK;
+}
+static int rh_carved_bytes(int ns, int nu, int n_pad, int H, size_t* out) {
+#define CALL(NS, NU) rh_carved_bytes<NS, NU>(n_pad, H, out)
+    SX_DISPATCH(ns, nu, CALL);
+#undef CALL
+}
+extern "C" long long sx_debug_rh_lds_bytes(int ns, int nu, int n_train, int n_pad, int H, int carved) {
+    size_t v = ~(size_t)0, rw = 0;
+    const int r = carved ? rh_carved_bytes(ns, nu, n_pad, H, &v) : resident_lds_bytes(ns, nu, n_train, n_pad, H, &v, &rw);
+    return r == SX_OK && v != ~(size_t)0 ? (long long)v : -1;
 }
 
 static RolloutPlan plan_rollout(const sx_gp_model* m, int sh, int H, bool elites, bool stream_only = false) {
diff --git a/safe_exploration_amd/csrc/sx_rollout_rh.hpp b/safe_exploration_amd/csrc/sx_rollout_rh.hpp
--- a/safe_exploration_amd/csrc/sx_rollout_rh.hpp
+++ b/safe_exploration_amd/csrc/sx_rollout_rh.hpp
@@ -19,14 +19,14 @@
 #ifndef SX_RH_PFL
 #define SX_RH_PFL 2
 #endif
-#ifndef SX_RH_RBMAJOR
-#define SX_RH_RBMAJOR 1
-#endif
-#ifndef SX_RH_PRIO
-#define SX_RH_PRIO 0
-#endif
-#ifndef SX_RH_WFIRST
-#define SX_RH_WFIRST 0
+#ifndef SX_RH_QSETUP
+#define SX_RH_QSETUP 1
+#endif
+#ifndef SX_RH_QPOLL
+#define SX_RH_QPOLL 256
+#endif
+#ifndef SX_RH_TOT
+#define SX_RH_TOT 1
 #endif
 #ifndef SX_RH_SHARES
 #define SX_RH_SHARES 4, 4, 4, 1, 4, 4, 4
@@ -78,6 +78,32 @@
             if (wave_of[d][rb] == w) return 2 * (rb + 1);
         return 0;
     }
+    constexpr int part_slot(int w, int d) const {
+        int s = 0;
+        for (int ww = 0; ww < kRhWaves; ++ww)
+            for (int dd = 0; dd < NS; ++dd) {
+                if (ww == w && dd == d) return s;
+                if (has(ww, dd)) ++s;
+            }
+        return s;
+    }
+    constexpr int part_slots() const { return part_slot(kRhWaves, 0); }
+    constexpr bool owns_mean_rows(int w) const {
+        for (int d = 0; d < NS; ++d)
+            for (int rb = NRB - 1; rb >= 0 && rb >= NRB - 2; --rb)
+                if (wave_of[d][rb] == w) return true;
+        return false;
+    }
+    constexpr int producer() const {
+        int best = -1;
+        for (int w = 0; w < kRhWaves; ++w) {
+            if (owns_mean_rows(w)) continue;
+            const int simd = pairs[w] + pairs[w ^ 4];
+            if (best < 0 || simd < pairs[best] + pairs[best ^ 4] || (simd == pairs[best] + pairs[best ^ 4] && pairs[w] < pairs[best]))
+                best = w;
+        }
+        return best;
+    }
 };
 
 template <int NS, int NRB>
@@ -90,15 +116,9 @@
         for (int w = 0; w < kRhWaves; ++w) {
             int idx = 0;
             for (int dd = 0; dd < NS; ++dd) {
-#if SX_RH_RBMAJOR
                 for (int r = NRB - 1; r >= 0; --r)
                     for (int qq = 0; qq < 2 * (r + 1); ++qq)
                         if (plan.wave_of[dd][r] == w) { d[w][idx] = dd; rb[w][idx] = r; q[w][idx] = qq; ++idx; }
-#else
-                for (int qq = 0; qq < 2 * NRB; ++qq)
-                    for (int r = NRB - 1; r >= 0; --r)
-                        if (plan.wave_of[dd][r] == w && qq < 2 * (r + 1)) { d[w][idx] = dd; rb[w][idx] = r; q[w][idx] = qq; ++idx; }
-#endif
             }
             n[w] = idx;
         }
@@ -162,32 +182,16 @@
         const int e_g0 = (SX_RH_LEAD < 0 || lay.ng == 0) ? lay.nr + lay.nl : lay.lead;
         const int e_l0 = (SX_RH_LEAD < 0 || lay.ng == 0) ? lay.nr : lay.lead + lay.ng;
         int bslot[RhElements<NS, NRB>::kMax] = {};
-        int bfirst[RhElements<NS, NRB>::kMax] = {};
-        int nloads = 0;
-        for (int e = 0; e < total; ++e) {
-            const bool fresh = SX_RH_RBMAJOR || e == 0 || el.q[WAVE][e] != el.q[WAVE][e - 1] || el.d[WAVE][e] != el.d[WAVE][e - 1];
-            if (fresh) ++nloads;
-            bfirst[e] = fresh ? 1 : 0;
-            bslot[e] = (nloads - 1) % (PF + 1);
-        }
+        for (int e = 0; e < total; ++e) bslot[e] = e % (PF + 1);
         constexpr int kDelay = 2;
         int pend_rb[NRB * NS] = {}, pend_d[NRB * NS] = {}, pend_at[NRB * NS] = {};
         int npend = 0, done = 0;
-        int issued_b = 0;
         int eb = 0;
         auto issue_b_upto = [&](int loads_wanted) {
-            while (issued_b < loads_wanted && eb < total) {
-                if (bfirst[eb]) {
-                    ops[n++] = RhOp{kRhLoadB, 0, 0, el.q[WAVE][eb], el.d[WAVE][eb], bslot[eb]};
-                    ++issued_b;
-                }
-                ++eb;
-            }
+            for (; eb < loads_wanted && eb < total; ++eb) ops[n++] = RhOp{kRhLoadB, 0, 0, el.q[WAVE][eb], el.d[WAVE][eb], bslot[eb]};
         };
-        int loads_seen = 0;
         for (int e = 0; e < total; ++e) {
-            if (bfirst[e]) ++loads_seen;
-            issue_b_upto(loads_seen + PF);
+            issue_b_upto(e + 1 + PF);
             while (next_l < lay.nl && e_l0 + next_l <= e + PFL) ops[n++] = RhOp{kRhLoadWL, REGP + next_l++, 0, 0, 0, 0};
             while (next_g < lay.ng && e_g0 + next_g <= e + PFG) ops[n++] = RhOp{kRhLoadWG, REGP + LDSP + next_g++, 0, 0, 0, 0};
             ops[n++] = RhOp{kRhMfma, lay.storage(e, REGP, LDSP), el.rb[WAVE][e], el.q[WAVE][e], el.d[WAVE][e], bslot[e], e};
@@ -213,9 +217,19 @@
     }
 };
 
+template <int NRB>
+__host__ __device__ constexpr int rh_flag_of(int d, int rb) {
+    return 2 * d + (NRB - 1 - rb);
+}
+template <int NS, int D>
+struct RhQuery {
+    static constexpr int kDoubles = (NS * (D + 1) + 1 + 1) & ~1;
+    static constexpr int kMark = NS * (D + 1);
+};
+
 template <int NS, int D, int NRB, int WAVE, int REGP, int LDSP>
 __device__ __forceinline__ void rh_mfma_phase(const GpConst<NS, D>& gc, GpTileLds<NS, D>& lds, const v2d* wlds_wave, int lane,
-                                              const v2d (&wreg)[REGP]) {
+                                              const v2d (&wreg)[REGP], int* qflag, int seq) {
     constexpr int PF = SX_RW_PF, PFL = SX_RH_PFL, PFG = SX_RH_PFG;
     constexpr int MAXP = RhPlan<NS, NRB>{}.max_pairs();
     static constexpr RhProgram<NS, NRB, WAVE, REGP, LDSP, PF, PFL, PFG> prog{};
@@ -243,10 +257,6 @@
         } else if constexpr (op.kind == kRhLoadWG) {
             wg[op.i % (PFG + 1)] = ap[(size_t)stream.pair[WAVE][op.i] * 64];
         } else if constexpr (op.kind == kRhMfma) {
-#if SX_RH_PRIO == 2
-            if constexpr ((4 * op.e) / prog.total != (4 * (op.e - 1)) / prog.total || op.e == 0)
-                __builtin_amdgcn_s_setprio(3 - (4 * op.e) / prog.total);
-#endif
             SX_PIN();
             const v2d bq = b[op.slot];
             v2d a;
@@ -276,36 +286,25 @@
                     else if (row - gc.n_train <= D)
                         lds.mj[d * 256 + (row - gc.n_train) * 16 + (lane & 15)] = acc[rb][r];
                 }
+#if SX_RH_QSETUP
+                asm volatile("s_waitcnt lgkmcnt(0)" ::: "memory");
+                if (lane == 0) *(volatile __attribute__((address_space(3))) int*)(qflag + rh_flag_of<NRB>(d, rb)) = seq;
+#endif
             } else {
                 s = fma(acc[rb][3], acc[rb][3], fma(acc[rb][2], acc[rb][2], fma(acc[rb][1], acc[rb][1], acc[rb][0] * acc[rb][0])));
             }
             ssq[d] += s;
         } else {
             constexpr int d = op.d;
+#if SX_RH_TOT
+            constexpr int slot = RhPlan<NS, NRB>{}.part_slot(WAVE, d);
+            lds.part[slot * 64 + lane] = ssq[d];
+#else
             const v4d tot = __builtin_amdgcn_mfma_f64_16x16x4f64(1.0, ssq[d], v4d{0.0, 0.0, 0.0, 0.0}, 0, 0, 0);
             if (lane < 16) lds.part[(WAVE * NS + d) * 16 + lane] = tot[0];
+#endif
         }
     });
-}
-
-template <int NS, int D, int NRB, bool WITH_JAC, typename G>
-__device__ __forceinline__ void rh_collect(const G& gc, const GpTileLds<NS, D>& lds, int c, const double (&z)[D],
-                                           double (&mean)[NS], double (&var)[NS], double (&jac)[NS][D]) {
-    constexpr RhPlan<NS, NRB> plan{};
-#pragma unroll
-    for (int d = 0; d < NS; ++d) {
-        double q = 0.0;
-#pragma unroll
-        for (int w = 0; w < kRhWaves; ++w)
-            if (plan.has(w, d)) q += lds.part[(w * NS + d) * 16 + c];
-        var[d] = (gc.outputscale[d] - q) + gc.noise[d];
-        const double m = lds.mj[d * 256 + c];
-        mean[d] = m;
-        if constexpr (WITH_JAC) {
-#pragma unroll
-            for (int j = 0; j < D; ++j) jac[d][j] = lds.mj[d * 256 + (1 + j) * 16 + c] - z[j] * gc.inv_ls2[d * D + j] * m;
-        }
-    }
 }
 
 template <int NS, int NRB>
@@ -321,10 +320,31 @@
 template <int NS, int NU, int NRB>
 inline size_t rh_lds_doubles(int n_train, int n_pad, int H) {
     constexpr int D = NS + NU, S = NS + NS * NS;
-    return (size_t)NS * n_pad * 16 + NS * 256 + (size_t)kRhWaves * NS * 16 + 32 * D + (((size_t)SX_TILE * H * NU + 1) & ~(size_t)1) +
-           (((size_t)SX_TILE * (2 * (S + NS) + 3) + 1) & ~(size_t)1) + RwKstarLds<NS, D>::doubles(n_pad) +
-           (size_t)kRhWaves * rh_ldsp<NS, NRB>() * 128;
+    return (size_t)NS * n_pad * 16 + NS * 256 + (SX_RH_TOT ? (size_t)RhPlan<NS, NRB>{}.part_slots() * 64 : (size_t)kRhWaves * NS * 16) + 32 * D +
+           (((size_t)SX_TILE * H * NU + 1) & ~(size_t)1) + (((size_t)SX_TILE * (2 * (S + NS) + 3) + 1) & ~(size_t)1) +
+           RwKstarLds<NS, D>::doubles(n_pad) + (size_t)kRhWaves * rh_ldsp<NS, NRB>() * 128 +
+           (SX_RH_QSETUP ? 2 * SX_TILE * RhQuery<NS, D>::kDoubles + ((NS + 1) & ~1) : 0);
 }
+
+template <int NS, int NU, int NRB>
+struct RhLdsMap {
+    static constexpr int D = NS + NU, S = NS + NS * NS;
+    size_t kfrag, mj, part, zs, acts, cst, pq, kstar, wlds, qrec, qflag, end;
+    __host__ __device__ RhLdsMap(int n_pad, int H) {
+        kfrag = 0;
+        mj = kfrag + (size_t)NS * n_pad * 16;
+        part = mj + NS * 256;
+        zs = part + (SX_RH_TOT ? (size_t)RhPlan<NS, NRB>{}.part_slots() * 64 : (size_t)kRhWaves * NS * 16);
+        acts = zs + 32 * D;
+        cst = acts + (((size_t)SX_TILE * H * NU + 1) & ~(size_t)1);
+        pq = cst + sizeof(RwConst<NS, NU>) / 8;
+        kstar = pq + (((size_t)SX_TILE * (2 * (S + NS) + 3) + 1) & ~(size_t)1);
+        wlds = kstar + RwKstarLds<NS, D>::doubles(n_pad);
+        qrec = wlds + (size_t)kRhWaves * rh_ldsp<NS, NRB>() * 128;
+        qflag = qrec + (SX_RH_QSETUP ? 2 * SX_TILE * RhQuery<NS, D>::kDoubles : 0);
+        end = qflag + (SX_RH_QSETUP ? (NS + 1) & ~1 : 0);
+    }
+};
 
 template <int NS, int NU, int NRB>
 __global__ __launch_bounds__(kRhThreads) void cem_rollout_rh_kernel(GpConst<NS, NS + NU> gc, ReachConst<NS, NU> rc,
@@ -341,36 +361,38 @@
     constexpr int nw = kRhWaves;
     lds.xs = nullptr;
     lds.etab = nullptr;
-    lds.kfrag = smem;
-    lds.mj = lds.kfrag + (size_t)NS * gc.n_pad * 16;
-    lds.part = lds.mj + NS * 256;
-    lds.zs = lds.part + (size_t)nw * NS * 16;
-    double* acts = lds.zs + 32 * D;
+    const RhLdsMap<NS, NU, NRB> map(gc.n_pad, rp.H);
+    lds.kfrag = smem + map.kfrag;
+    lds.mj = smem + map.mj;
+    lds.part = smem + map.part;
+    lds.zs = smem + map.zs;
+    double* acts = smem + map.acts;
     const int tid = threadIdx.x;
     const int wave = __builtin_amdgcn_readfirstlane(tid >> 6), lane = tid & 63;
     const int H = rp.H;
     const int tiles_per_problem = (rp.P + SX_TILE - 1) / SX_TILE;
     const int total_tiles = rp.E * tiles_per_problem;
 
-    RwConst<NS, NU>* const cst = reinterpret_cast<RwConst<NS, NU>*>(acts + (((size_t)SX_TILE * rp.H * NU + 1) & ~(size_t)1));
-    double* const pq = reinterpret_cast<double*>(cst + 1);
+    RwConst<NS, NU>* const cst = reinterpret_cast<RwConst<NS, NU>*>(smem + map.cst);
+    double* const pq = smem + map.pq;
     RwKstarLds<NS, D> kl;
-    kl.carve(pq + (((size_t)SX_TILE * (2 * PQS + 3) + 1) & ~(size_t)1), gc.n_pad);
-    v2d* const wlds = reinterpret_cast<v2d*>(kl.xbar + ((D + 1) & ~1));
+    kl.carve(smem + map.kstar, gc.n_pad);
+    v2d* const wlds = reinterpret_cast<v2d*>(smem + map.wlds);
+#if SX_RH_QSETUP
+    typedef RhQuery<NS, D> QR;
+    constexpr int kProducer = plan.producer();
+    static_assert(kProducer >= 0 && !plan.owns_mean_rows(kProducer), "a wave without a mean-row block makes the query set-up");
+    double* const qrec = smem + map.qrec;
+    int* const qflag = reinterpret_cast<int*>(smem + map.qflag);
+    if (threadIdx.x < 2 * NS) qflag[threadIdx.x] = 0;
+    const bool two_blocks = NRB > 1 && (gc.n_train >> 4) < NRB - 1;
+#else
+    int* const qflag = nullptr;
+#endif
+    int seq = 0;
 
     static constexpr RhStream<NS, NRB, MAXP, REGP, LDSP> stream{};
     v2d wreg[REGP];
-#if SX_RH_WFIRST
-    {
-        const v2d* __restrict__ const ap0 = reinterpret_cast<const v2d*>(gc.a_pack) + lane;
-#pragma unroll
-        for (int i = 0; i < REGP; ++i) wreg[i] = ap0[(size_t)stream.pair[wave][i] * 64];
-        if constexpr (LDSP > 0) {
-#pragma unroll
-            for (int i = 0; i < LDSP; ++i) wlds[(wave * LDSP + i) * 64 + lane] = ap0[(size_t)stream.pair[wave][REGP + i] * 64];
-        }
-    }
-#endif
     {
         static_assert(sizeof(RwConst<NS, NU>) % 8 == 0 && sizeof(ReachConst<NS, NU>) % 8 == 0 &&
                       sizeof(CostConst<SX_MAX_M, NS, NU>) % 8 == 0, "copied in 8-byte words");
@@ -485,7 +507,7 @@
         }
         __syncthreads();
 
-        if (!SX_RH_WFIRST && tile == (int)blockIdx.x) {
+        if (tile == (int)blockIdx.x) {
             const v2d* __restrict__ const ap = reinterpret_cast<const v2d*>(gc.a_pack) + lane;
             if constexpr (LDSP > 0) {
                 const __amdgpu_buffer_rsrc_t arsrc =
@@ -516,14 +538,41 @@
             double z[D], u[NU], mean[NS], var[NS], jac[NS][D], p1[NS], Q1[NS][NS];
             double p[NS], Q[NS][NS];
             constexpr RhPlan<NS, NRB> plan{};
-            const double* my = st_row(t & 1, lane);
+#if SX_RH_QSETUP
+            int ln = lane;
+            asm volatile("" : "+v"(ln));
+#else
+            const int ln = lane;
+#endif
+            const double* my = st_row(t & 1, ln);
             double partv[NS][kRhWaves], mjv[NS][1 + D], ils2[NS][D], osc[NS], nzv[NS];
+#if SX_RH_TOT
+            {
+                double partq[NS][kRhWaves][4];
+#pragma unroll
+                for (int d = 0; d < NS; ++d)
+#pragma unroll
+                    for (int w = 0; w < kRhWaves; ++w)
+#pragma unroll
+                        for (int k = 0; k < 4; ++k)
+                            partq[d][w][k] = plan.has(w, d) ? lds.part[plan.part_slot(w, d) * 64 + 16 * k + ln] : 0.0;
+                SX_PIN();
+#pragma unroll
+                for (int d = 0; d < NS; ++d)
+#pragma unroll
+                    for (int w = 0; w < kRhWaves; ++w)
+                        partv[d][w] = ((partq[d][w][0] + partq[d][w][1]) + partq[d][w][2]) + partq[d][w][3];
+                SX_PIN();
+            }
+#endif
 #pragma unroll
             for (int d = 0; d < NS; ++d) {
-#pragma unroll
-                for (int w = 0; w < kRhWaves; ++w) partv[d][w] = plan.has(w, d) ? lds.part[(w * NS + d) * 16 + lane] : 0.0;
-#pragma unroll
-                for (int r = 0; r < 1 + D; ++r) mjv[d][r] = lds.mj[d * 256 + r * 16 + lane];
+#if !SX_RH_TOT
+#pragma unroll
+                for (int w = 0; w < kRhWaves; ++w) partv[d][w] = plan.has(w, d) ? lds.part[(w * NS + d) * 16 + ln] : 0.0;
+#endif
+#pragma unroll
+                for (int r = 0; r < 1 + D; ++r) mjv[d][r] = lds.mj[d * 256 + r * 16 + ln];
             }
 #pragma unroll
             for (int i = 0; i < NS; ++i) {
@@ -532,7 +581,7 @@
                 for (int j = 0; j < NS; ++j) Q[i][j] = my[NS + i * NS + j];
             }
 #pragma unroll
-            for (int cidx = 0; cidx < NU; ++cidx) u[cidx] = acts[(lane * H + t) * NU + cidx];
+            for (int cidx = 0; cidx < NU; ++cidx) u[cidx] = acts[(ln * H + t) * NU + cidx];
 #pragma unroll
             for (int d = 0; d < NS; ++d) {
                 osc[d] = fc.outputscale[d];
@@ -580,15 +629,15 @@
                     p1[i] = sc;
                 }
                 if (t + 1 < H) {
-                    double* zn = zs_base + ((t + 1) & 1) * 16 * D + lane * D;
+                    double* zn = zs_base + ((t + 1) & 1) * 16 * D + ln * D;
 #pragma unroll
                     for (int i = 0; i < NS; ++i) zn[i] = p1[i];
 #pragma unroll
-                    for (int cidx = 0; cidx < NU; ++cidx) zn[NS + cidx] = acts[(lane * H + t + 1) * NU + cidx];
+                    for (int cidx = 0; cidx < NU; ++cidx) zn[NS + cidx] = acts[(ln * H + t + 1) * NU + cidx];
                 }
             }
             if (lane_valid && st_step) reinterpret_cast<int*>(ac_row + 2)[0] |= st_step;
-            double* nx = st_row((t + 1) & 1, lane);
+            double* nx = st_row((t + 1) & 1, ln);
 #pragma unroll
             for (int i = 0; i < NS; ++i) {
                 nx[i] = p1[i];
@@ -684,6 +733,7 @@
 
 #ifdef SX_STAMPS
         unsigned long long c_k = 0, c_kb = 0, c_m = 0, c_mb = 0;
+        unsigned long long c_head = 0, c_prod = 0, c_price = 0;
         unsigned long long rt0;
         asm volatile("s_memrealtime %0\n\ts_waitcnt lgkmcnt(0)" : "=s"(rt0)::"memory");
         const unsigned long long ct0 = stamp();
@@ -693,7 +743,61 @@
             const unsigned long long t0 = stamp();
 #endif
             const bool kstar_wave = !(t > 0 && wave == 0);
+            ++seq;
             if (wave == 4 && t > 1) finish_costs(t - 2);
+#ifdef SX_STAMPS
+            const unsigned long long tp1 = stamp();
+            c_price += tp1 - t0;
+#endif
+#if SX_RH_QSETUP
+            if (kstar_wave) {
+                double zq[D];
+                RwKstarQuery<NS, D> qs;
+                const int c = lane & 15;
+                bool produced = false;
+                if (t > 0) {
+                    int cq = lane;
+                    asm volatile("" : "+v"(cq));
+                    const v2d* r2 = reinterpret_cast<const v2d*>(qrec + ((t & 1) * SX_TILE + (cq & 15)) * QR::kDoubles);
+                    double rv[QR::kDoubles];
+#pragma unroll
+                    for (int i = 0; i < QR::kDoubles / 2; ++i) {
+                        const v2d v = r2[i];
+                        rv[2 * i] = v.x;
+                        rv[2 * i + 1] = v.y;
+                    }
+                    const int mark = __builtin_amdgcn_readfirstlane((int)rv[QR::kMark]);
+                    produced = mark != 2;
+#pragma unroll
+                    for (int d = 0; d < NS; ++d) {
+                        qs.zz[d] = rv[d];
+#pragma unroll
+                        for (int j = 0; j < D; ++j) qs.g[d][j] = rv[NS + d * D + j];
+                    }
+                    qs.znan = rv[QR::kMark] != 0.0;
+                }
+                if (!produced) {
+                    if (t == 0) {
+#pragma unroll
+                        for (int j = 0; j < D; ++j) zq[j] = zs_base[c * D + j];
+                    } else {
+                        double pc[NS];
+                        next_centre(rc, c, zs_base + ((t - 1) & 1) * 16 * D + c * D, pc);
+#pragma unroll
+                        for (int i = 0; i < NS; ++i) zq[i] = pc[i];
+#pragma unroll
+                        for (int cidx = 0; cidx < NU; ++cidx) zq[NS + cidx] = acts[(c * H + t) * NU + cidx];
+                    }
+                    rw_kstar_query(gc, kl, zq, qs.zz, qs.g, qs.znan);
+                }
+#ifdef SX_STAMPS
+                c_head += stamp() - tp1;
+#endif
+                rw_kstar_phase<NS, D, true>(gc, kl, lds.kfrag, t == 0 ? q0_begin : q_begin, t == 0 ? q0_end : q_end, zq, &qs);
+            } else if (owner) {
+                finish_state(t - 1);
+            }
+#else
             if (kstar_wave) {
                 double zq[D];
                 const int c = lane & 15;
@@ -713,6 +817,7 @@
             } else if (owner) {
                 finish_state(t - 1);
             }
+#endif
 #ifdef SX_STAMPS
             const unsigned long long t1 = stamp();
 #endif
@@ -722,26 +827,61 @@
             const unsigned long long t2 = stamp();
 #endif
             const v2d* wl = wlds + wave * LDSP * 64;
-#if SX_RH_PRIO == 1
-            if (wave < 4) __builtin_amdgcn_s_setprio(3);
-#endif
             switch (wave) {
-                case 0: rh_mfma_phase<NS, D, NRB, 0, REGP, LDSP>(gc, lds, wl, lane, wreg); break;
-                case 1: rh_mfma_phase<NS, D, NRB, 1, REGP, LDSP>(gc, lds, wl, lane, wreg); break;
-                case 2: rh_mfma_phase<NS, D, NRB, 2, REGP, LDSP>(gc, lds, wl, lane, wreg); break;
-                case 3: rh_mfma_phase<NS, D, NRB, 3, REGP, LDSP>(gc, lds, wl, lane, wreg); break;
-                case 4: rh_mfma_phase<NS, D, NRB, 4, REGP, LDSP>(gc, lds, wl, lane, wreg); break;
-                case 5: rh_mfma_phase<NS, D, NRB, 5, REGP, LDSP>(gc, lds, wl, lane, wreg); break;
-                case 6: rh_mfma_phase<NS, D, NRB, 6, REGP, LDSP>(gc, lds, wl, lane, wreg); break;
-                default: rh_mfma_phase<NS, D, NRB, 7, REGP, LDSP>(gc, lds, wl, lane, wreg); break;
-            }
-#if SX_RH_PRIO == 1
-            if (wave < 4) __builtin_amdgcn_s_setprio(0);
-#elif SX_RH_PRIO == 2
-            __builtin_amdgcn_s_setprio(0);
-#endif
+                case 0: rh_mfma_phase<NS, D, NRB, 0, REGP, LDSP>(gc, lds, wl, lane, wreg, qflag, seq); break;
+                case 1: rh_mfma_phase<NS, D, NRB, 1, REGP, LDSP>(gc, lds, wl, lane, wreg, qflag, seq); break;
+                case 2: rh_mfma_phase<NS, D, NRB, 2, REGP, LDSP>(gc, lds, wl, lane, wreg, qflag, seq); break;
+                case 3: rh_mfma_phase<NS, D, NRB, 3, REGP, LDSP>(gc, lds, wl, lane, wreg, qflag, seq); break;
+                case 4: rh_mfma_phase<NS, D, NRB, 4, REGP, LDSP>(gc, lds, wl, lane, wreg, qflag, seq); break;
+                case 5: rh_mfma_phase<NS, D, NRB, 5, REGP, LDSP>(gc, lds, wl, lane, wreg, qflag, seq); break;
+                case 6: rh_mfma_phase<NS, D, NRB, 6, REGP, LDSP>(gc, lds, wl, lane, wreg, qflag, seq); break;
+                default: rh_mfma_phase<NS, D, NRB, 7, REGP, LDSP>(gc, lds, wl, lane, wreg, qflag, seq); break;
+            }
 #ifdef SX_STAMPS
             const unsigned long long t3 = stamp();
+#endif
+#if SX_RH_QSETUP
+            if (wave == kProducer && t + 1 < H) {
+                typedef volatile __attribute__((address_space(3))) int* lflag;
+                bool ready = false;
+                for (int i = 0; i < SX_RH_QPOLL && !ready; ++i) {
+                    ready = true;
+#pragma unroll
+                    for (int d = 0; d < NS; ++d) {
+                        ready = ready && *(lflag)(qflag + rh_flag_of<NRB>(d, NRB - 1)) == seq;
+                        if (NRB > 1 && two_blocks) ready = ready && *(lflag)(qflag + rh_flag_of<NRB>(d, NRB - 2)) == seq;
+                    }
+                    if (!ready) __builtin_amdgcn_s_sleep(1);
+                }
+                asm volatile("" ::: "memory");
+                if (lane_owner) {
+                    int c = lane;
+                    asm volatile("" : "+v"(c));
+                    double* rec = qrec + (((t + 1) & 1) * SX_TILE + c) * QR::kDoubles;
+                    if (ready) {
+                        double zq[D], pc[NS];
+                        RwKstarQuery<NS, D> qs;
+                        next_centre(rc, c, zs_base + (t & 1) * 16 * D + c * D, pc);
+#pragma unroll
+                        for (int i = 0; i < NS; ++i) zq[i] = pc[i];
+#pragma unroll
+                        for (int cidx = 0; cidx < NU; ++cidx) zq[NS + cidx] = acts[(c * H + t + 1) * NU + cidx];
+                        rw_kstar_query(gc, kl, zq, qs.zz, qs.g, qs.znan);
+#pragma unroll
+                        for (int d = 0; d < NS; ++d) {
+                            rec[d] = qs.zz[d];
+#pragma unroll
+                            for (int j = 0; j < D; ++j) rec[NS + d * D + j] = qs.g[d][j];
+                        }
+                        rec[QR::kMark] = qs.znan ? 1.0 : 0.0;
+                    } else {
+                        rec[QR::kMark] = 2.0;
+                    }
+                }
+            }
+#ifdef SX_STAMPS
+            c_prod += stamp() - t3;
+#endif
 #endif
             __syncthreads();
 #ifdef SX_STAMPS
@@ -754,7 +894,7 @@
         const unsigned long long loop_t1 = stamp();
         if (rp.stamps && lane == 0 && tile == (int)blockIdx.x) {
             unsigned long long* o = rp.stamps + ((size_t)blockIdx.x * nw + wave) * 8;
-            o[0] = c_k; o[1] = c_kb; o[2] = c_m; o[3] = c_mb;
+            o[0] = c_k | (c_head << 32); o[1] = c_kb | (c_prod << 32); o[2] = c_m | (c_price << 32); o[3] = c_mb;
             o[4] = (ct0 - tile_t0) | (first_k << 32);
             unsigned long long rt1;
             asm volatile("s_memrealtime %0\n\ts_waitcnt lgkmcnt(0)" : "=s"(rt1)::"memory");
diff --git a/safe_exploration_amd/csrc/sx_rollout_rw.hpp b/safe_exploration_amd/csrc/sx_rollout_rw.hpp
--- a/safe_exploration_amd/csrc/sx_rollout_rw.hpp
+++ b/safe_exploration_amd/csrc/sx_rollout_rw.hpp
@@ -223,8 +223,38 @@
 }
 
 template <int NS, int D>
+__device__ __forceinline__ void rw_kstar_query(const GpConst<NS, D>& gc, const RwKstarLds<NS, D>& kl, const double (&z)[D],
+                                               double (&zz)[NS], double (&g)[NS][D], bool& znan) {
+    double zc[D];
+    znan = false;
+#pragma unroll
+    for (int j = 0; j < D; ++j) {
+        zc[j] = z[j] - kl.xbar[j];
+        znan = znan || (z[j] != z[j]);
+    }
+#pragma unroll
+    for (int d = 0; d < NS; ++d) {
+        double a = gc.k_log_os[d];
+#pragma unroll
+        for (int j = 0; j < D; ++j) {
+            const double kz = gc.k_nh_ils2[d * D + j] * zc[j];
+            a = fma(kz, zc[j], a);
+            g[d][j] = -2.0 * kz;
+        }
+        zz[d] = a;
+    }
+}
+
+template <int NS, int D>
+struct RwKstarQuery {
+    double zz[NS], g[NS][D];
+    bool znan;
+};
+
+template <int NS, int D, bool PRE = false>
 __device__ __forceinline__ void rw_kstar_phase(const GpConst<NS, D>& gc, const RwKstarLds<NS, D>& kl, double* kfrag,
-                                               int q_begin, int q_end, const double (&z)[D]) {
+                                               int q_begin, int q_end, const double (&z)[D],
+                                               const RwKstarQuery<NS, D>* pre = nullptr) {
     constexpr int M = 2 * NS, RS = D + NS;
     const int n = q_end - q_begin;
     if (n <= 0) return;
@@ -232,24 +262,16 @@
     const int c = lane & 15;
     double zz[NS], g[NS][D];
     bool znan = false;
-    {
-        double zc[D];
-#pragma unroll
-        for (int j = 0; j < D; ++j) {
-            zc[j] = z[j] - kl.xbar[j];
-            znan = znan || (z[j] != z[j]);
-        }
+    if constexpr (PRE) {
 #pragma unroll
         for (int d = 0; d < NS; ++d) {
-            double a = gc.k_log_os[d];
-#pragma unroll
-            for (int j = 0; j < D; ++j) {
-                const double kz = gc.k_nh_ils2[d * D + j] * zc[j];
-                a = fma(kz, zc[j], a);
-                g[d][j] = -2.0 * kz;
-            }
-            zz[d] = a;
-        }
+            zz[d] = pre->zz[d];
+#pragma unroll
+            for (int j = 0; j < D; ++j) g[d][j] = pre->g[d][j];
+        }
+        znan = pre->znan;
+    } else {
+        rw_kstar_query(gc, kl, z, zz, g, znan);
     }
     const lds_f64* etab = (const lds_f64*)kl.tab + (znan ? kExpTab2 : 0);
     const int emask = znan ? 0 : kExpTab2 - 1;
diff --git a/safe_exploration_amd/csrc/sx_rw_impl.hpp b/safe_exploration_amd/csrc/sx_rw_impl.hpp
--- a/safe_exploration_amd/csrc/sx_rw_impl.hpp
+++ b/safe_exploration_amd/csrc/sx_rw_impl.hpp
@@ -22,6 +22,13 @@
 size_t rollout_rh_lds_bytes(int n_train, int n_pad, int H) {
     return with_nrb<rh_max_nrb(NS, NU)>(n_pad >> 4, ~(size_t)0, [&](auto nrb_c) {
         return rh_lds_doubles<NS, NU, decltype(nrb_c)::value>(n_train, n_pad, H) * sizeof(double) + sizeof(RwConst<NS, NU>);
+    });
+}
+
+template <int NS, int NU>
+size_t rollout_rh_carved_bytes(int n_pad, int H) {
+    return with_nrb<rh_max_nrb(NS, NU)>(n_pad >> 4, ~(size_t)0, [&](auto nrb_c) {
+        return RhLdsMap<NS, NU, decltype(nrb_c)::value>(n_pad, H).end * sizeof(double);
     });
 }
 
@@ -79,6 +86,7 @@
 
 #define SX_RW_INSTANTIATE(NS, NU)                                                                                         \
     template size_t rollout_rh_lds_bytes<NS, NU>(int, int, int);                                                          \
+    template size_t rollout_rh_carved_bytes<NS, NU>(int, int);                                                            \
     template size_t rollout_rw_lds_bytes<NS, NU>(int, int, int);                                                          \
     template int launch_rollout_rh<NS, NU>(const GpConst<NS, NS + NU>&, const ReachConst<NS, NU>&,                        \
                                            const CostConst<SX_MAX_M, NS, NU>&, const RolloutPtrs&, int, size_t, hipStream_t); \
diff --git a/safe_exploration_amd/csrc/sx_rw_launch.hpp b/safe_exploration_amd/csrc/sx_rw_launch.hpp
--- a/safe_exploration_amd/csrc/sx_rw_launch.hpp
+++ b/safe_exploration_amd/csrc/sx_rw_launch.hpp
@@ -21,6 +21,8 @@
 size_t rollout_rh_lds_bytes(int n_train, int n_pad, int H);
 template <int NS, int NU>
 size_t rollout_rw_lds_bytes(int n_train, int n_pad, int H);
+template <int NS, int NU>
+size_t rollout_rh_carved_bytes(int n_pad, int H);
 
 template <int NS, int NU>
 int launch_rollout_rh(const GpConst<NS, NS + NU>& gc, const ReachConst<NS, NU>& rc, const CostConst<SX_MAX_M, NS, NU>& cc,
```

New measurement: 467.5 million (median of 6 runs). No clear change (+0.7%).
